# submarine0418/underwater_image_enhancement

Measured on AMD Instinct MI355X. Metric: megapixels/sec enhanced, higher is better.
Workload: dtype f32/f64

## Files before the change

include/uwie.h:

```cpp
#ifndef UWIE_H_
#define UWIE_H_

#include <stddef.h>
#include <stdint.h>

#ifdef __cplusplus
extern "C" {
#endif

#define UWIE_OK 0
#define UWIE_E_INVALID (-1)
#define UWIE_E_WORKSPACE (-2)
#define UWIE_E_HIP (-3)
#define UWIE_E_NODEVICE (-4)
#define UWIE_E_DEVICE (-5)

#define UWIE_SURFACE_SIX 0
#define UWIE_SURFACE_DICT 1

#define UWIE_DICT_STRONG_DEHAZING 0
#define UWIE_DICT_MEDIUM_DEHAZING 1
#define UWIE_DICT_LIGHT_ENHANCEMENT 2
#define UWIE_DICT_CLAHE_ENHANCEMENT 3
#define UWIE_DICT_HISTOGRAM_EQUALIZATION 4

#define UWIE_CAST_NORMAL 0
#define UWIE_CAST_GREENISH 1
#define UWIE_CAST_BLUISH 2

typedef struct uwie_ctx uwie_ctx;

typedef struct uwie_params {
    int32_t surface;
    int32_t strategy;
    int32_t cast_correct;
    int32_t forced_cast;
    int32_t gray_shift;
    int32_t min_size;
    double omega;
    int32_t gf_ksize;
    double gf_eps;
    double L_low, L_high;
    double wb_percentile;
    double clip_limit;
    int32_t tiles_x, tiles_y;
    double gamma;
    int32_t apply_gamma;
    int32_t gf_exact;
    int32_t inter_dtype;
    int32_t dark_patch;
} uwie_params;

#define UWIE_INTER_F64 0
#define UWIE_INTER_FX32 1
#define UWIE_INTER_F32T 2

const char *uwie_last_error(void);
const char *uwie_version(void);

int uwie_create(int device, uwie_ctx **out_ctx);
void uwie_destroy(uwie_ctx *ctx);

#define UWIE_STATUS_CANNY_LABEL 1u
#define UWIE_STATUS_FALLBACK_SYNC 2u
#define UWIE_STATUS_QTREE_BOUNDS 4u
#define UWIE_STATUS_FEATURE_COUNTS 8u
#define UWIE_STATUS_DIFF_RANK 16u
#define UWIE_STATUS_RESIZE_DESC 32u
#define UWIE_STATUS_CLASSIFY_NAN 64u
int uwie_device_status(uwie_ctx *ctx, void *stream, uint32_t *bits);

int uwie_profile_enable(uwie_ctx *ctx, int on);
int uwie_profile_filter(uwie_ctx *ctx, const char *kernel_name);
int uwie_profile_collect(uwie_ctx *ctx);
int uwie_profile_row(uwie_ctx *ctx, int i, const char **name, double *total_ms, int *calls);

int uwie_params_init(uwie_params *p, int surface, int strategy);

int uwie_set_tuning(uwie_ctx *ctx, const char *name, int value);
int uwie_get_tuning(uwie_ctx *ctx, const char *name, int *value);

size_t uwie_workspace_bytes(int batch, int H, int W, const uwie_params *p);
size_t uwie_workspace_bytes_ctx(uwie_ctx *ctx, int batch, int H, int W, const uwie_params *p);

int uwie_enhance_u8(uwie_ctx *ctx, const uint8_t *d_in, uint8_t *d_out_u8, float *d_out_f32, int batch, int H, int W,
                    const uwie_params *p, void *d_workspace, size_t workspace_bytes, void *stream);

int uwie_enhance_u8_f64(uwie_ctx *ctx, const uint8_t *d_in, uint8_t *d_out_u8, double *d_out_f64, int batch, int H, int W,
                        const uwie_params *p, void *d_workspace, size_t workspace_bytes, void *stream);

int uwie_enhance_percentiles(uwie_ctx *ctx, const void *d_workspace, size_t workspace_bytes, int batch, int H, int W,
                             const uwie_params *p, double *d_out, void *stream);

size_t uwie_workspace_bytes_float(int batch, int H, int W, const uwie_params *p, int elem_bytes);
int uwie_enhance_f32(uwie_ctx *ctx, const float *d_img, uint8_t *d_out_u8, float *d_out_f32, double *d_out_f64, int batch, int H, int W,
                     const uwie_params *p, void *d_workspace, size_t workspace_bytes, void *stream);
int uwie_enhance_f64(uwie_ctx *ctx, const double *d_img, uint8_t *d_out_u8, double *d_out_f64, int batch, int H, int W,
                     const uwie_params *p, void *d_workspace, size_t workspace_bytes, void *stream);
int uwie_cast_classify_f32(uwie_ctx *ctx, const float *d_img, int batch, int H, int W, int32_t *d_kind, float *d_mean_rgb, void *stream);
int uwie_color_correct_f32(uwie_ctx *ctx, const float *d_img, const int32_t *d_kind, float *d_out, int batch, int H, int W, void *stream);

size_t uwie_workspace_bytes_all(int batch, int H, int W, const uwie_params *p6);

int uwie_enhance_all_u8(uwie_ctx *ctx, const uint8_t *d_in, uint8_t *d_out_u8, int32_t *d_kind, int batch, int H, int W,
                        const uwie_params *p6, void *d_workspace, size_t workspace_bytes, void *stream);

#define UWIE_DIFF_OMEGA 1
#define UWIE_DIFF_GAMMA 2
int uwie_diff_enhance_f32(uwie_ctx *ctx, const float *d_img, float *d_out, int batch, int H, int W, int planar,
                          const float *d_params, int flags, void *d_workspace, size_t workspace_bytes, void *stream);

int uwie_diff_enhance_save_f32(uwie_ctx *ctx, const float *d_img, float *d_out, int batch, int H, int W, int planar,
                               const float *d_params, int flags, float *d_saved, void *d_workspace, size_t workspace_bytes,
                               void *stream);
size_t uwie_diff_enhance_bwd_workspace_bytes(int batch, int H, int W);
int uwie_diff_enhance_bwd_f32(uwie_ctx *ctx, const float *d_img, const float *d_params, int flags, int planar, int batch,
                              int H, int W, const float *d_saved, const float *d_grad_out, float *d_grad_img,
                              float *d_grad_params, void *d_workspace, size_t workspace_bytes, void *stream);

size_t uwie_workspace_bytes_diff_u8(int batch, int H, int W);
int uwie_diff_enhance_u8(uwie_ctx *ctx, const uint8_t *d_in, uint8_t *d_out_u8, float *d_out_f32, int batch, int H, int W,
                         const float *d_params ,
                         int flags , float *d_saved , void *d_workspace,
                         size_t workspace_bytes, void *stream);

int uwie_diff_gated_f32(uwie_ctx *ctx, const float *d_img, float *d_out, int batch, int H, int W, int planar,
                        const float *d_params, int flags, void *d_workspace, size_t workspace_bytes, void *stream);
int uwie_diff_gated_save_f32(uwie_ctx *ctx, const float *d_img, float *d_out, int batch, int H, int W, int planar,
                             const float *d_params, int flags, float *d_saved, void *d_workspace, size_t workspace_bytes,
                             void *stream);
size_t uwie_diff_gated_bwd_workspace_bytes(int batch, int H, int W);
int uwie_diff_gated_bwd_f32(uwie_ctx *ctx, const float *d_img, const float *d_params, int flags, int planar, int batch, int H,
                            int W, const float *d_saved, const float *d_grad_out, float *d_grad_img, float *d_grad_params,
                            void *d_workspace, size_t workspace_bytes, void *stream);

size_t uwie_workspace_bytes_diff_gated_u8(int batch);
int uwie_diff_gated_u8(uwie_ctx *ctx, const uint8_t *d_in, uint8_t *d_out_u8, float *d_out_f32, int batch, int H, int W,
                       const float *d_params , int flags ,
                       float *d_saved , void *d_workspace, size_t workspace_bytes, void *stream);

#define UWIE_LOSS_IDENTITY 0
#define UWIE_LOSS_VGG 1
#define UWIE_LOSS_GATED 2
size_t uwie_ref_loss_workspace_bytes(int batch, int H, int W);
int uwie_ref_loss_f32(uwie_ctx *ctx, int map, const float *d_img, const float *d_params, int flags, int planar, int batch, int H,
                      int W, const float *d_ref, float *d_out, float *d_saved, float *d_loss, void *d_workspace,
                      size_t workspace_bytes, void *stream);
int uwie_ref_loss_bwd_f32(uwie_ctx *ctx, int map, const float *d_img, const float *d_params, int flags, int planar, int batch,
                          int H, int W, const float *d_saved, const float *d_ref, const float *d_grad_out,
                          const float *d_grad_loss, float *d_grad_img, float *d_grad_params, void *d_workspace,
                          size_t workspace_bytes, void *stream);
int uwie_device_status_async(uwie_ctx *ctx, uint32_t *d_bits, void *stream);

// ... 207 lines not shown
```

underwater_image_enhancement_amd/_lib.py:

```python
from __future__ import annotations

import ctypes
import os
import subprocess

_HERE = os.path.dirname(os.path.abspath(__file__))
LIB_PATH = os.path.join(_HERE, "lib", "libuwie.so")
CSRC = os.path.join(_HERE, "csrc")

SURFACE_SIX, SURFACE_DICT = 0, 1
STATUS_DIFF_RANK = 16
STATUS_CLASSIFY_NAN = 64
LOSS_IDENTITY, LOSS_VGG, LOSS_GATED = 0, 1, 2
VGG_F32, VGG_F16, VGG_PARAMS = 0, 1, 1735488
PARAM_NET_PARAMS = {True: 8500100, False: 8459652}
MASKS_GIVEN, MASKS_DRAWN = 0, 1
TRAINER_PARAMS, TRAINER_GRADS, TRAINER_EXP_AVG, TRAINER_EXP_AVG_SQ = 0, 1, 2, 3
FLIP_LR, FLIP_UD = 1, 2
RESIZE_MAX_SIDE, RESIZE_MAX_SRC = 4096, 32768
INTER_F64, INTER_FX32, INTER_F32T = 0, 1, 2
DICT_STRATEGIES = {
    "strong_dehazing": 0,
    "medium_dehazing": 1,
    "light_enhancement": 2,
# ... 36 lines not shown
class UwieModelDesc(ctypes.Structure):

    _fields_ = [("kind", ctypes.c_int32), ("n_features", ctypes.c_int32), ("n_classes", ctypes.c_int32),
                ("n_trees", ctypes.c_int32), ("n_nodes", ctypes.c_int32), ("n_sv", ctypes.c_int32),
                ("mean", ctypes.c_void_p), ("scale", ctypes.c_void_p),
                ("tree_offset", ctypes.c_void_p), ("left", ctypes.c_void_p), ("right", ctypes.c_void_p),
                ("feature", ctypes.c_void_p), ("threshold", ctypes.c_void_p), ("missing_left", ctypes.c_void_p),
                ("value", ctypes.c_void_p), ("learning_rate", ctypes.c_double), ("init", ctypes.c_void_p),
                ("sv", ctypes.c_void_p), ("dual_coef", ctypes.c_void_p), ("intercept", ctypes.c_void_p),
                ("n_support", ctypes.c_void_p), ("prob_a", ctypes.c_void_p), ("prob_b", ctypes.c_void_p),
                ("gamma", ctypes.c_double)]


class UwieClahePlan(ctypes.Structure):

    _fields_ = [(name, ctypes.c_int32) for name in ("tile_w", "tile_h", "padded", "clip_limit", "wide_lut", "nchunk",
                                                    "cells_walk", "cells_flat")]


def clahe_plan(batch, H, W, tiles=(8, 8), clip_limit=2.0, recomputed=False) -> UwieClahePlan:
    out = UwieClahePlan()
    check(load().uwie_clahe_plan(batch, H, W, int(tiles[0]), int(tiles[1]), float(clip_limit), int(bool(recomputed)),
                                 ctypes.byref(out)))
    return out


def dark_patch_plan(H, W, k) -> tuple[int, int]:
    tw, th = ctypes.c_int(), ctypes.c_int()
    check(load().uwie_dark_patch_plan(int(H), int(W), int(k), ctypes.byref(tw), ctypes.byref(th)))
    return tw.value, th.value


UW_SCORES = 8


def underwater_plan(H, W) -> tuple[int, int]:
    tw, th = ctypes.c_int(), ctypes.c_int()
    check(load().uwie_underwater_plan(int(H), int(W), ctypes.byref(tw), ctypes.byref(th)))
    return tw.value, th.value


REF_SCORES = 8


def reference_plan(H, W) -> tuple[int, int]:
    tw, th = ctypes.c_int(), ctypes.c_int()
    check(load().uwie_reference_plan(int(H), int(W), ctypes.byref(tw), ctypes.byref(th)))
    return tw.value, th.value


GW_STATS = 12


def gray_world_plan(H, W) -> tuple[int, int]:
    bp, tp = ctypes.c_int(), ctypes.c_int()
    check(load().uwie_gray_world_plan(int(H), int(W), ctypes.byref(bp), ctypes.byref(tp)))
    return bp.value, tp.value


def fusion_plan(H, W, levels=1) -> tuple[int, int]:
    tw, th = ctypes.c_int(), ctypes.c_int()
    check(load().uwie_fusion_plan(int(H), int(W), int(levels), ctypes.byref(tw), ctypes.byref(th)))
    return tw.value, th.value


def fusion_table(gamma):
    import numpy as np

    buf = (ctypes.c_uint8 * 256)()
    check(load().uwie_fusion_table(float(gamma), buf))
    return np.frombuffer(bytes(buf), dtype=np.uint8).copy()


_VP, _SZ, _I, _D = ctypes.c_void_p, ctypes.c_size_t, ctypes.c_int, ctypes.c_double
_PP = ctypes.POINTER(UwieParams)
_PM = ctypes.POINTER(UwieModelDesc)
_PI = ctypes.POINTER(_I)
SIGNATURES = {
    "uwie_last_error": [],
    "uwie_version": [],
    "uwie_create": [_I, ctypes.POINTER(_VP)],
    "uwie_destroy": [_VP],
    "uwie_device_status": [_VP, _VP, ctypes.POINTER(ctypes.c_uint32)],
    "uwie_profile_enable": [_VP, _I],
    "uwie_profile_filter": [_VP, ctypes.c_char_p],
    "uwie_profile_collect": [_VP],
    "uwie_profile_row": [_VP, _I, ctypes.POINTER(ctypes.c_char_p), ctypes.POINTER(_D), ctypes.POINTER(_I)],
    "uwie_params_init": [_PP, _I, _I],
    "uwie_set_tuning": [_VP, ctypes.c_char_p, _I],
    "uwie_get_tuning": [_VP, ctypes.c_char_p, ctypes.POINTER(_I)],
    "uwie_workspace_bytes": [_I, _I, _I, _PP],
    "uwie_workspace_bytes_ctx": [_VP, _I, _I, _I, _PP],
    "uwie_workspace_bytes_all": [_I, _I, _I, _VP],
    "uwie_workspace_bytes_float": [_I, _I, _I, _PP, _I],
    "uwie_enhance_f32": [_VP, _VP, _VP, _VP, _VP, _I, _I, _I, _PP, _VP, _SZ, _VP],
    "uwie_enhance_f64": [_VP, _VP, _VP, _VP, _I, _I, _I, _PP, _VP, _SZ, _VP],
    "uwie_cast_classify_f32": [_VP, _VP, _I, _I, _I, _VP, _VP, _VP],
    "uwie_color_correct_f32": [_VP, _VP, _VP, _VP, _I, _I, _I, _VP],
    "uwie_guided_plan": [_I, _I, _I, _I, ctypes.POINTER(ctypes.c_int), ctypes.POINTER(ctypes.c_int)],
    "uwie_guided_fill": [_I, _I, _I, _I, ctypes.POINTER(ctypes.c_longlong)],
    "uwie_clahe_plan": [_I, _I, _I, _I, _I, _D, _I, ctypes.POINTER(UwieClahePlan)],
    "uwie_dark_patch_plan": [_I, _I, _I, ctypes.POINTER(ctypes.c_int), ctypes.POINTER(ctypes.c_int)],
    "uwie_enhance_u8": [_VP, _VP, _VP, _VP, _I, _I, _I, _PP, _VP, _SZ, _VP],
    "uwie_enhance_u8_f64": [_VP, _VP, _VP, _VP, _I, _I, _I, _PP, _VP, _SZ, _VP],
    "uwie_enhance_percentiles": [_VP, _VP, _SZ, _I, _I, _I, _PP, _VP, _VP],
    "uwie_enhance_all_u8": [_VP, _VP, _VP, _VP, _I, _I, _I, _VP, _VP, _SZ, _VP],
    "uwie_workspace_bytes_select": [_I, _I, _I, _VP, _I, _I],
    "uwie_select_best_u8": [_VP, _VP, _I, _I, _I, _VP, _I, _VP, _VP, _VP, _VP, _VP, _VP, _SZ, _VP],
    "uwie_workspace_bytes_underwater": [_I, _I, _I],
    "uwie_underwater_plan": [_I, _I, ctypes.POINTER(ctypes.c_int), ctypes.POINTER(ctypes.c_int)],
    "uwie_underwater_scores_u8": [_VP, _VP, _I, _I, _I, _I, _VP, _VP, _SZ, _VP],
    "uwie_workspace_bytes_reference": [_I, _I, _I],
    "uwie_reference_plan": [_I, _I, ctypes.POINTER(ctypes.c_int), ctypes.POINTER(ctypes.c_int)],
    "uwie_reference_scores_u8": [_VP, _VP, _VP, _I, _I, _I, _I, _I, _VP, _VP, _SZ, _VP],
    "uwie_workspace_bytes_gray_world": [_I, _I, _I],
    "uwie_gray_world_plan": [_I, _I, ctypes.POINTER(ctypes.c_int), ctypes.POINTER(ctypes.c_int)],
    "uwie_gray_world_u8": [_VP, _VP, _I, _I, _I, _D, _D, _D, _VP, _VP, _VP, _SZ, _VP],
    "uwie_workspace_bytes_fusion": [_I, _I, _I, _I],
    "uwie_fusion_plan": [_I, _I, _I, ctypes.POINTER(ctypes.c_int), ctypes.POINTER(ctypes.c_int)],
    "uwie_fusion_table": [_D, ctypes.POINTER(ctypes.c_uint8)],
    "uwie_fusion_u8": [_VP, _VP, _I, _I, _I, _D, _I, _I, _VP, _VP, _VP, _VP, _VP, _SZ, _VP],
    "uwie_pick_best_u8": [_VP, _VP, _I, _I, _I, _I, _VP, _I, _I, _VP, _VP, _VP],
    "uwie_diff_enhance_f32": [_VP, _VP, _VP, _I, _I, _I, _I, _VP, _I, _VP, _SZ, _VP],
    "uwie_diff_enhance_save_f32": [_VP, _VP, _VP, _I, _I, _I, _I, _VP, _I, _VP, _VP, _SZ, _VP],
    "uwie_diff_enhance_bwd_workspace_bytes": [_I, _I, _I],
    "uwie_workspace_bytes_diff_u8": [_I, _I, _I],
    "uwie_diff_enhance_u8": [_VP, _VP, _VP, _VP, _I, _I, _I, _VP, _I, _VP, _VP, _SZ, _VP],
    "uwie_diff_enhance_bwd_f32": [_VP, _VP, _VP, _I, _I, _I, _I, _I, _VP, _VP, _VP, _VP, _VP, _SZ, _VP],
    "uwie_diff_gated_f32": [_VP, _VP, _VP, _I, _I, _I, _I, _VP, _I, _VP, _SZ, _VP],
    "uwie_diff_gated_save_f32": [_VP, _VP, _VP, _I, _I, _I, _I, _VP, _I, _VP, _VP, _SZ, _VP],
    "uwie_diff_gated_bwd_workspace_bytes": [_I, _I, _I],
    "uwie_workspace_bytes_diff_gated_u8": [_I],
    "uwie_diff_gated_u8": [_VP, _VP, _VP, _VP, _I, _I, _I, _VP, _I, _VP, _VP, _SZ, _VP],
    "uwie_diff_gated_bwd_f32": [_VP, _VP, _VP, _I, _I, _I, _I, _I, _VP, _VP, _VP, _VP, _VP, _SZ, _VP],
    "uwie_ref_loss_workspace_bytes": [_I, _I, _I],
    "uwie_ref_loss_f32": [_VP, _I, _VP, _VP, _I, _I, _I, _I, _I, _VP, _VP, _VP, _VP, _VP, _SZ, _VP],
    "uwie_ref_loss_bwd_f32": [_VP, _I, _VP, _VP, _I, _I, _I, _I, _I, _VP, _VP, _VP, _VP, _VP, _VP, _VP, _SZ, _VP],
    "uwie_device_status_async": [_VP, _VP, _VP],
    "uwie_vgg_create": [_VP, _VP, _I, ctypes.POINTER(_VP)],
    "uwie_vgg_destroy": [_VP],
    "uwie_perceptual_workspace_bytes": [_I, _I, _I, _I],
    "uwie_perceptual_f32": [_VP, _VP, _VP, _VP, _I, _I, _I, _VP, _VP, _SZ, _VP],
    "uwie_perceptual_bwd_f32": [_VP, _VP, _I, _I, _I, _VP, _VP, _VP, _SZ, _VP],
    "uwie_param_net_create": [_VP, _VP, _I, ctypes.POINTER(_VP)],
    "uwie_param_net_destroy": [_VP],
    "uwie_param_net_workspace_bytes": [_I, _I, _I],
    "uwie_param_net_f32": [_VP, _VP, _VP, _VP, _I, _I, _I, _VP, _VP, _VP, _SZ, _VP],
    "uwie_mlp_create": [_VP, _VP, _I, _I, _I, ctypes.POINTER(_VP)],
    "uwie_mlp_destroy": [_VP],
    "uwie_mlp_workspace_bytes": [_I, _I],
    "uwie_mlp_forward": [_VP, _VP, _VP, _I, _I, _VP, _VP, _SZ, _VP],
    "uwie_mlp_trainer_create": [_VP, _VP, _I, _I, _I, ctypes.POINTER(_VP)],
    "uwie_mlp_trainer_destroy": [_VP],
    "uwie_mlp_train_workspace_bytes": [_I, _I, _I],
    "uwie_mlp_train_forward": [_VP, _VP, _VP, _I, _I, _D, _I, _VP, ctypes.c_uint64, _VP, _VP, _SZ, _VP],
    "uwie_mlp_backward": [_VP, _VP, _VP, _I, _I, _VP, _VP, _SZ, _VP],
    "uwie_mlp_adam_step": [_VP, _VP, _D, _D, _D, _D, _D, _VP, _VP],
    "uwie_mlp_trainer_get": [_VP, _I, _VP],
    "uwie_mlp_trainer_set": [_VP, _I, _VP],
    "uwie_mlp_trainer_step_count": [_VP],
    "uwie_mlp_trainer_set_step_count": [_VP, ctypes.c_longlong],
    "uwie_mlp_trainer_eval": [_VP, _VP, _VP, _I, _I, _VP, _VP, _SZ, _VP],
    "uwie_u8_to_f32": [_VP, _VP, _VP, _SZ, _VP],
    "uwie_extract_features_u8": [_VP, _VP, _VP, _I, _I, _I, _VP, _SZ, _VP],
    "uwie_feature_extractor_count": [_I, _I],
    "uwie_workspace_bytes_feature_extractor": [_I, _I, _I],
# ... 92 lines not shown
```

underwater_image_enhancement_amd/csrc/api.hip:

```cpp
#include <algorithm>
#include <cmath>
#include <cstdarg>
#include <cstdio>
#include <cstring>
#include <type_traits>

#include "common.h"

#include <cstdlib>

namespace uwie {

static thread_local char g_err[512] = "";
static thread_local uwie_ctx *g_ctx = nullptr;
static const Tuning g_default_tuning{};

const Tuning &tune() { return g_ctx ? g_ctx->tune : g_default_tuning; }
uwie_ctx *current_ctx() { return g_ctx; }

void set_error(const char *fmt, ...)
{
    va_list ap;
    va_start(ap, fmt);
    vsnprintf(g_err, sizeof g_err, fmt, ap);
// ... 191 lines not shown
    }
    size_scratch(u, s);
    return u;
}

Pipe carve_pipe(Carver &c, Shape s, const EnhancePlan &e)
{
    Pipe P{};
    const size_t n = (size_t)s.B * s.npx();
    P.kind = c.take<int32_t>(s.B);
    P.A = c.take<float>((size_t)s.B * 3);
    P.pct = c.take<float>((size_t)s.B * 3 * kMaxPct);
    P.guess = c.take<int32_t>(s.B);
    if (e.F64) {
        P.F64 = c.take<double>(n * 3);
        P.pct64 = c.take<double>((size_t)s.B * 3 * kMaxPct);
    }
    if (e.F) P.F = c.take<float>(n * 3);
    if (e.dehaze) {
        P.gray = c.take<uint8_t>(n);
        if (!e.t0_in_scratch) P.t0 = c.take<float>(n);
        P.t = c.take<double>(n);
    }
    P.scratch_bytes = e.scratch_bytes;
    P.scratch = c.take<char>(P.scratch_bytes);
    P.planes = e.guided.planes;
    if (e.t0_in_scratch) P.t0 = static_cast<float *>(P.scratch);
    if (e.qpart && P.scratch) P.qpart = reinterpret_cast<uint32_t *>(static_cast<char *>(P.scratch) + e.qoff);
    return P;
}

int stage_guided(const Pipe &P, Shape s, const EnhancePlan &e, const FuseT0Args &frame, hipStream_t st)
{
    const GuidedPlan &g = e.guided;
    UWIE_REQUIRE(!g.planes || (P.planes && P.t0 != P.scratch), "guided filter: the workspace layout has no planes for the exact-order filter");
    if (g.t0) UWIE_TRY(launch_t0(frame, e.dark_patch, s, P.t0, st));
    return launch_guided_plan(g, s, P.gray, P.t0, P.t, P.scratch, st, &frame);
}

int stretch_f32(const float *img, float *out, Shape s, double lo, double hi, float eps, float *pct, void *ws, hipStream_t st)
{
    const double q[2] = {lo, hi};
    UWIE_TRY(launch_percentiles(img, 0, s, q, 2, pct, ws, st));
    return launch_stretch_apply_f32(img, pct, 2, 0, 1, eps, out, s, st);
}

int six_cast(uwie_ctx *ctx, const uint8_t *d_in, Shape s, const EnhancePlan &e, const uwie_params *p, const Pipe &P,
             const int32_t **kind, hipStream_t st)
{
    *kind = nullptr;
    if (p->forced_cast >= 0) {
        UWIE_TRY(launch_set_kind(P.kind, s.B, p->forced_cast, st));
        *kind = P.kind;
    } else if (p->cast_correct) {
        const EntryFuse ef{P.qpart, e.cast_gray ? P.gray : nullptr, P.guess, p->gray_shift};
        UWIE_TRY(launch_cast_classify(ctx, d_in, s, P.kind, nullptr, P.scratch, st, e.qpart ? &ef : nullptr));
        *kind = P.kind;
    }
    return UWIE_OK;
}

int six_airlight(uwie_ctx *ctx, const uint8_t *d_in, const int32_t *kind, Shape s, const EnhancePlan &e, const uwie_params *p,
                 const Pipe &P, hipStream_t st)
{
    return launch_airlight(ctx, d_in, kind, P.gray, s, p->min_size, P.A, nullptr, P.scratch, st, e.cast_gray ? 0 : p->gray_shift,
                           e.qpart ? P.qpart : nullptr);
}

int six_dehaze_tail(uwie_ctx *ctx, const uint8_t *d_in, const int32_t *kind, Shape s, const EnhancePlan &e, const uwie_params *p,
                    const Pipe &P, uint8_t *d_out_u8, float *d_out_f32, hipStream_t st)
{
    const float eps = 1e-6f;
    const int k = p->strategy, nq = k == 3 ? 4 : 2, t_is_f32 = e.guided.t_f32;
    UWIE_TRY(stage_guided(P, s, e, FuseT0Args{d_in, kind, P.A, (float)p->omega, 1e-6f, 1}, st));
    SelectPlan plan;
    const double q[4] = {p->L_low, p->L_high, p->wb_percentile, 100 - p->wb_percentile};
    const RestoreSrc src{d_in, kind, P.A, P.t, t_is_f32};
    const RestoreSrc *recompute = e.store ? nullptr : &src;
    if (e.generic) {
        UWIE_TRY(select_begin<float>(s, q, nq, P.scratch, st, &plan));
        UWIE_TRY(launch_restore_planar_hist(d_in, kind, P.A, P.t, s, P.F, plan.ghist, st, false, nullptr, t_is_f32));
        UWIE_TRY(select_run(plan, P.F, 1, s, true, st));
    } else {
        UWIE_TRY(select_lin_begin<float>(s, q, nq, P.scratch, st, &plan, e.predict ? &src : nullptr));
        if (e.rank && plan.predicted) {
            UWIE_TRY(launch_restore_rank(src, s, plan, st));
            UWIE_TRY(select_rank_run(plan, s, st, src));
        } else {
            UWIE_TRY(launch_restore_planar_hist(d_in, kind, P.A, P.t, s, e.store ? P.F : nullptr, plan.ghist, st, true, &plan, t_is_f32));
            UWIE_TRY(select_lin_run(plan, P.F, s, st, recompute));
        }
    }
    if (k == 3) {
        UWIE_TRY(select_lerp_chain(plan, s, eps, P.pct, st));
        return launch_tail_plain(P.F, P.pct, 4, eps, 1, s, 0, 1.0, d_out_u8, d_out_f32, st);
    }
    UWIE_TRY(select_lerp(plan, s, P.pct, st));
    return launch_tail_clahe(ctx, P.F, P.pct, 2, eps, 0, s, p->clip_limit, e.tx, e.ty, k == 1 ? 1 : 0, p->gamma, d_out_u8, d_out_f32,
                             P.scratch, st, recompute);
}

int dict_dehaze(uwie_ctx *ctx, const uint8_t *d_in, Shape s, const EnhancePlan &e, const uwie_params *p, const Pipe &P,
                uint8_t *d_out_u8, float *d_out_f32, double *d_out_f64, hipStream_t st, bool have_airlight)
{
    if (!have_airlight)
        UWIE_TRY(launch_airlight(ctx, d_in, nullptr, P.gray, s, p->min_size, P.A, nullptr, P.scratch, st, p->gray_shift));
    UWIE_TRY(stage_guided(P, s, e, FuseT0Args{d_in, nullptr, P.A, (float)p->omega, 1e-10f, 0}, st));
    SelectPlan plan;
    const double q[2] = {p->L_low, p->L_high};
    const RestoreSrc src{d_in, nullptr, P.A, P.t};
    const RestoreSrc *recompute = e.store ? nullptr : &src;
    if (e.generic) {
        UWIE_TRY(select_begin<double>(s, q, 2, P.scratch, st, &plan));
        UWIE_TRY(launch_recover64_planar_hist(d_in, P.A, P.t, s, P.F64, plan.ghist, st));
        UWIE_TRY(select_run(plan, P.F64, 1, s, true, st));
    } else {
        UWIE_TRY(select_lin_begin<double>(s, q, 2, P.scratch, st, &plan, &src));
        UWIE_TRY(launch_recover64_planar_hist(d_in, P.A, P.t, s, e.store ? P.F64 : nullptr, plan.ghist, st, true, &plan));
        UWIE_TRY(select_lin_run(plan, P.F64, s, st, recompute));
    }
    UWIE_TRY(select_lerp(plan, s, P.pct64, st));
    return launch_tail_plain64(P.F64, P.pct64, s, p->apply_gamma, p->gamma, d_out_u8, d_out_f32, st, recompute, d_out_f64);
}

int run_enhance(uwie_ctx *ctx, const uint8_t *d_in, Shape s, const EnhancePlan &e, const uwie_params *p, const Pipe &P,
                uint8_t *d_out_u8, float *d_out_f32, double *d_out_f64, hipStream_t st, bool have_airlight = false)
{
    const int32_t *kind = nullptr;
    switch (e.pipeline) {
    case EP_SIX_DEHAZE:
        UWIE_TRY(six_cast(ctx, d_in, s, e, p, P, &kind, st));
        UWIE_TRY(six_airlight(ctx, d_in, kind, s, e, p, P, st));
        return six_dehaze_tail(ctx, d_in, kind, s, e, p, P, d_out_u8, d_out_f32, st);
    case EP_SIX_CODES:
        UWIE_TRY(six_cast(ctx, d_in, s, e, p, P, &kind, st));
        return launch_code_strategy(ctx, d_in, kind, s, p, d_out_u8, d_out_f32, P.scratch, st);
    case EP_DICT_DEHAZE: return dict_dehaze(ctx, d_in, s, e, p, P, d_out_u8, d_out_f32, d_out_f64, st, have_airlight);
    default: return launch_code_strategy(ctx, d_in, nullptr, s, p, d_out_u8, d_out_f32, P.scratch, st, d_out_f64);
    }
}

int check_params(const uwie_params *p)
{
    UWIE_REQUIRE(p != nullptr, "params is NULL");
    UWIE_REQUIRE(p->surface == UWIE_SURFACE_SIX || p->surface == UWIE_SURFACE_DICT, "unknown surface");
    if (p->surface == UWIE_SURFACE_SIX) UWIE_REQUIRE(p->strategy >= 1 && p->strategy <= 6, "unknown strategy");
    else UWIE_REQUIRE(p->strategy >= 0 && p->strategy <= 4, "unknown strategy");
    UWIE_REQUIRE(p->gray_shift == 14 || p->gray_shift == 15, "gray_shift must be 14 or 15");
    UWIE_REQUIRE(p->forced_cast >= -1 && p->forced_cast <= 2, "forced_cast must be -1 or a UWIE_CAST_* kind");
    UWIE_REQUIRE(p->min_size >= 1, "min_size must be >= 1");
    UWIE_REQUIRE(p->tiles_x >= 1 && p->tiles_y >= 1 && p->tiles_x * p->tiles_y <= 4096, "bad CLAHE tile grid");
    if (dehazes(p)) UWIE_REQUIRE(p->gf_ksize >= 1 && p->gf_ksize <= 1024, "guided-filter width out of range");
    UWIE_REQUIRE(p->L_low >= 0.0 && p->L_low <= 100.0 && p->L_high >= 0.0 && p->L_high <= 100.0,
                 "L_low / L_high must be percentiles in [0, 100]");
    if (p->surface == UWIE_SURFACE_SIX && (p->strategy >= 3 && p->strategy <= 5))
        UWIE_REQUIRE(p->wb_percentile >= 0.0 && p->wb_percentile <= 100.0, "wb_percentile must be in [0, 100]");
    UWIE_REQUIRE(p->inter_dtype == UWIE_INTER_F64 || p->inter_dtype == UWIE_INTER_FX32 || p->inter_dtype == UWIE_INTER_F32T,
                 "unknown inter_dtype");
    UWIE_REQUIRE(p->dark_patch >= 0 && p->dark_patch <= 31, "dark_patch must be 0 .. 31 (0 and 1: the per-pixel dark channel)");
    return UWIE_OK;
}


template <class T>
struct FloatPipe {
    int32_t *kind;
    T *A;
    float *pct;
// ... 211 lines not shown
const char *uwie_version(void) { return "uwie 0.1 (gfx950)"; }

int uwie_create(int device, uwie_ctx **out_ctx)
{
    UWIE_REQUIRE(out_ctx != nullptr, "out_ctx is NULL");
    *out_ctx = nullptr;
    int count = 0;
    if (hipGetDeviceCount(&count) != hipSuccess || count <= 0) {
        set_error("no HIP device available (libuwie has no CPU path)");
        return UWIE_E_NODEVICE;
    }
    UWIE_REQUIRE(device >= 0 && device < count, "device index out of range");
    UWIE_HIP_CHECK(hipSetDevice(device));
    int cus = 0;
    UWIE_HIP_CHECK(hipDeviceGetAttribute(&cus, hipDeviceAttributeMultiprocessorCount, device));
    uwie_ctx *ctx = new uwie_ctx();
    ctx->aux_ready = false;
    ctx->prof = prof_create();
    ctx->device = device;
    ctx->cus = cus;
    tuning_from_env(&ctx->tune);
    LabTables *lab = new LabTables();
    CastTables *cast = new CastTables();
    build_lab_tables(lab);
    build_cast_tables(cast);
    hipError_t e = hipMalloc((void **)&ctx->d_lab, sizeof(LabTables));
    if (e == hipSuccess) e = hipMalloc((void **)&ctx->d_cast, sizeof(CastTables));
    if (e == hipSuccess) e = hipMalloc((void **)&ctx->d_status, 64);
    if (e == hipSuccess) e = hipMemset(ctx->d_status, 0, 64);
    if (e == hipSuccess) e = hipMemcpy(ctx->d_lab, lab, sizeof(LabTables), hipMemcpyHostToDevice);
    if (e == hipSuccess) e = hipMemcpy(ctx->d_cast, cast, sizeof(CastTables), hipMemcpyHostToDevice);
    delete lab;
    delete cast;
    if (e != hipSuccess) {
        set_error("context table upload failed: %s", hipGetErrorString(e));
        uwie_destroy(ctx);
        return UWIE_E_HIP;
    }
    *out_ctx = ctx;
    return UWIE_OK;
}

void uwie_destroy(uwie_ctx *ctx)
{
    if (!ctx) return;
    if (ctx->d_lab) (void)hipFree(ctx->d_lab);
    if (ctx->d_cast) (void)hipFree(ctx->d_cast);
    if (ctx->d_status) (void)hipFree(ctx->d_status);
    if (ctx->aux_ready) {
        for (int i = 0; i < 4; ++i) {
            (void)hipStreamDestroy(ctx->aux[i]);
            (void)hipEventDestroy(ctx->join[i]);
        }
        (void)hipEventDestroy(ctx->fork);
    }
    prof_bind(nullptr);
    prof_destroy(ctx->prof);
    delete ctx;
}

int uwie_device_status(uwie_ctx *ctx, void *stream, uint32_t *bits)
{
    UWIE_REQUIRE(ctx != nullptr, "device_status: NULL context");
    UWIE_SCOPE(ctx);
    uint32_t v = 0;
    hipStream_t st = (hipStream_t)stream;
    UWIE_HIP_CHECK(hipMemcpyAsync(&v, ctx->d_status, sizeof v, hipMemcpyDeviceToHost, st));
    UWIE_HIP_CHECK(hipStreamSynchronize(st));
    if (v) UWIE_HIP_CHECK(hipMemsetAsync(ctx->d_status, 0, sizeof v, st));
    if (bits) *bits = v;
    if (v) {
        set_error("device status 0x%x:%s the results of the calls since the last check are not valid", v,
                  (v & UWIE_STATUS_CANNY_LABEL) ? " Canny hysteresis met a component label that this launch did not write (k_canny.hip);"
                  : (v & UWIE_STATUS_QTREE_BOUNDS) ? " a quadtree score fell outside its histogram interval (k_airlight.hip, tuning q_hist = 3);"
                  : (v & UWIE_STATUS_FEATURE_COUNTS) ? " a frame's feature histograms do not count every pixel (k_extractor.hip);"
                  : (v & UWIE_STATUS_DIFF_RANK) ? " a gated DifferentiableEnhancement image has no valid sorted position (an IndexError, ValueError or OverflowError in Python);"
                  : (v & UWIE_STATUS_RESIZE_DESC) ? " a resize frame descriptor has a NULL pointer or a size out of range (k_resize.hip);"
                  : (v & UWIE_STATUS_CLASSIFY_NAN) ? " a row holds NaN and the model is GB or SVC (scikit-learn: ValueError, Input X contains NaN);" : "");
        return UWIE_E_DEVICE;
    }
    return UWIE_OK;
}

int uwie_device_status_async(uwie_ctx *ctx, uint32_t *d_bits, void *stream)
{
    UWIE_REQUIRE(ctx && d_bits, "device_status_async: NULL pointer");
    UWIE_SCOPE(ctx);
    hipStream_t st = (hipStream_t)stream;
    UWIE_HIP_CHECK(hipMemcpyAsync(d_bits, ctx->d_status, sizeof(uint32_t), hipMemcpyDeviceToDevice, st));
    UWIE_HIP_CHECK(hipMemsetAsync(ctx->d_status, 0, sizeof(uint32_t), st));
    return UWIE_OK;
}

int uwie_profile_enable(uwie_ctx *ctx, int on)
{
    UWIE_REQUIRE(ctx != nullptr, "profile_enable: NULL context");
    prof_enable(ctx->prof, on != 0);
    prof_bind(on ? ctx->prof : nullptr);
    return UWIE_OK;
}

int uwie_profile_filter(uwie_ctx *ctx, const char *kernel_name)
{
    UWIE_REQUIRE(ctx != nullptr, "ctx is NULL");
    prof_filter(ctx->prof, kernel_name);
    return UWIE_OK;
}

int uwie_profile_collect(uwie_ctx *ctx)
{
    if (!ctx) {
        set_error("profile_collect: NULL context");
        return UWIE_E_INVALID;
    }
    return prof_collect(ctx->prof);
}

int uwie_profile_row(uwie_ctx *ctx, int i, const char **name, double *total_ms, int *calls)
{
    UWIE_REQUIRE(ctx && name && total_ms && calls, "profile_row: NULL pointer");
    return prof_row(ctx->prof, i, name, total_ms, calls);
}

int uwie_set_tuning(uwie_ctx *ctx, const char *name, int value)
{
    UWIE_REQUIRE(ctx && name, "set_tuning: NULL pointer");
    for (const KnobName &k : kKnobs)
        if (std::strcmp(k.name, name) == 0) {
            ctx->tune.*(k.field) = value;
            return UWIE_OK;
        }
    set_error("set_tuning: unknown selector '%s'", name);
    return UWIE_E_INVALID;
}

int uwie_get_tuning(uwie_ctx *ctx, const char *name, int *value)
{
    UWIE_REQUIRE(ctx && name && value, "get_tuning: NULL pointer");
    for (const KnobName &k : kKnobs)
        if (std::strcmp(k.name, name) == 0) {
            *value = ctx->tune.*(k.field);
            return UWIE_OK;
        }
    set_error("get_tuning: unknown selector '%s'", name);
    return UWIE_E_INVALID;
}

int uwie_params_init(uwie_params *p, int surface, int strategy)
{
    UWIE_REQUIRE(p != nullptr, "params is NULL");
    std::memset(p, 0, sizeof *p);
    p->surface = surface;
    p->strategy = strategy;
    p->gray_shift = 15;
    p->min_size = 1;
    p->tiles_x = p->tiles_y = 8;
    p->wb_percentile = -1.0;
    p->gamma = 1.2;
    p->forced_cast = -1;
    p->dark_patch = 1;
    if (surface == UWIE_SURFACE_SIX) {
        p->cast_correct = 1;
        switch (strategy) {
        case 1: p->omega = 0.3; p->gf_ksize = 20; p->gf_eps = 5e-1; p->L_low = 5; p->L_high = 98; p->clip_limit = 3.0; p->gamma = 1.5; p->apply_gamma = 1; break;
        case 2: p->omega = 0.5; p->gf_ksize = 15; p->gf_eps = 5e-1; p->L_low = 15; p->L_high = 95; p->clip_limit = 2.0; break;
        case 3: p->omega = 0.7; p->gf_ksize = 10; p->gf_eps = 1e-1; p->L_low = 20; p->L_high = 85; p->wb_percentile = 2; break;
// ... 1455 lines not shown
```

underwater_image_enhancement_amd/csrc/common.h:

```cpp
#pragma once
#include <hip/hip_runtime.h>
#include <stddef.h>
#include <stdint.h>

#include "../../include/uwie.h"

namespace uwie {

void set_error(const char *fmt, ...);
#define UWIE_HIP_CHECK(expr)                                                            \
    do {                                                                                \
        hipError_t _e = (expr);                                                         \
        if (_e != hipSuccess) {                                                         \
            ::uwie::set_error("%s failed: %s (%s:%d)", #expr, hipGetErrorString(_e), __FILE__, __LINE__); \
            return UWIE_E_HIP;                                                          \
        }                                                                               \
    } while (0)
#define UWIE_LAUNCH_CHECK() UWIE_HIP_CHECK(hipGetLastError())
#define UWIE_REQUIRE(cond, msg)                 \
    do {                                        \
        if (!(cond)) {                          \
            ::uwie::set_error("%s", msg);       \
            return UWIE_E_INVALID;              \
        }                                       \
    } while (0)

constexpr int kCastBinadeMin = -2;
constexpr int kCastBinades = 34;

struct LabTables {
    uint16_t gamma[256];
    uint16_t cbrt[3072];
    int32_t fwd[9];
    uint8_t invgamma[4096];
    int32_t ltoyf[512];
    int32_t abtoxz[36864];
    int32_t inv[9];
};

struct CastTables {
    uint32_t R[kCastBinades][256];
    uint8_t tie[kCastBinades][256];
    uint32_t RT[256][kCastBinades];
    uint2 RT2[128][kCastBinades];
    uint8_t tiebin[256];
};

void build_lab_tables(LabTables *t);
void build_cast_tables(CastTables *t);

struct Profiler;
Profiler *prof_create();
void prof_destroy(Profiler *p);
void prof_enable(Profiler *p, bool on);
void prof_filter(Profiler *p, const char *name);
void prof_bind(Profiler *p);
int prof_collect(Profiler *p);
int prof_row(Profiler *p, int i, const char **name, double *ms, int *calls);
class ProfScope {
public:
    ProfScope(const char *name, hipStream_t st);
    ~ProfScope();
    ProfScope(const ProfScope &) = delete;

private:
    int rec_;
    hipStream_t st_;
};
#define UWIE_PROF_CAT2(a, b) a##b
#define UWIE_PROF_CAT(a, b) UWIE_PROF_CAT2(a, b)
#define UWIE_PROF(name, st) ::uwie::ProfScope UWIE_PROF_CAT(_uwie_prof_, __LINE__)(name, st)
#define UWIE_LAUNCH_AS(row, kernel, grid, block, lds, st, ...)              \
    do {                                                                    \
        UWIE_PROF(row, st);                                                 \
        hipLaunchKernelGGL(kernel, grid, block, lds, st, __VA_ARGS__);      \
    } while (0)
#define UWIE_LAUNCH(kernel, ...) UWIE_LAUNCH_AS(#kernel, kernel, __VA_ARGS__)

}

namespace uwie {
struct Tuning {
    int gf_split = 1;
    int gf_bands = 0;
    int select_generic = 0;
    int restore_store = 0;
    int lin_predict3 = 0;
    int lin_cap = 0;
    int lin_no_predict = 0;
    int q_hist = 1;
    int lin_predict_shift = 0;
    int streams = 1;
    int canny_prepass = 1;
    int gf_fuse = 2;
    int rank_sweep = 1;
    int canny_fault_inject = 0;
    int entry_fuse = 1;
};
const Tuning &tune();
uwie_ctx *current_ctx();
}

struct uwie_ctx {
    int device;
    uwie::Tuning tune;
    bool attr_q_tail = false;
    bool attr_cast_resolve = false;
    int attr_gf_fast = 0;
    int attr_gf_split8 = 0;
    int cus = 0;
    uwie::LabTables *d_lab;
    uwie::CastTables *d_cast;
    uwie::Profiler *prof;
    uint32_t *d_status = nullptr;
    hipStream_t aux[4];
    hipEvent_t fork, join[4];
    bool aux_ready;
    bool last_enhance_f64 = false;
};

namespace uwie {

struct Carver {
    char *base;
    size_t off;
    explicit Carver(void *b) : base(static_cast<char *>(b)), off(0) {}
    template <typename T>
    T *take(size_t count)
    {
        off = (off + 255) & ~size_t(255);
        T *p = base ? reinterpret_cast<T *>(base + off) : nullptr;
        off += count * sizeof(T);
        return p;
    }
    size_t total() const { return (off + 255) & ~size_t(255); }
};

static inline int cdiv(long long a, long long b) { return (int)((a + b - 1) / b); }
static inline int grid_for(size_t n, size_t cap = 8192)
{
    size_t g = (n + 255) / 256;
    if (g > cap) g = cap;
    return g < 1 ? 1 : (int)g;
}

struct Region {
    int32_t img, y0, x0, rows, cols;
};

struct Shape {
    int B, H, W;
    size_t npx() const { return (size_t)H * W; }
};

size_t cast_ws_bytes(Shape s);
struct EntryFuse {
    uint32_t *qpart;
    uint8_t *gray;
    int32_t *guess;
    int gray_shift;
};
int launch_cast_classify(uwie_ctx *ctx, const uint8_t *d_in, Shape s, int32_t *d_kind, float *d_mean, void *ws,
                         hipStream_t st, const EntryFuse *ef = nullptr);
size_t quad_part_bytes(Shape s);
int launch_quad_hist_reduce(const uint32_t *qpart, Shape s, uint32_t *d_hist, hipStream_t st);
int launch_set_kind(int32_t *d_kind, int B, int kind, hipStream_t st);
int launch_normalise_correct(const uint8_t *d_in, const int32_t *d_kind, float *d_out, Shape s, hipStream_t st);
int launch_quant_gray(const uint8_t *d_in, const int32_t *d_kind, uint8_t *d_gray, Shape s, int gray_shift,
                      hipStream_t st);

size_t airlight_ws_bytes(Shape s);
int launch_airlight(uwie_ctx *ctx, const uint8_t *d_in, const int32_t *d_kind, uint8_t *d_gray, Shape s, int min_size,
                    float *d_A, void *d_trace, void *ws, hipStream_t st, int make_gray_shift = 0, const uint32_t *qpart = nullptr);
bool entry_fuse_takes(Shape s, int min_size);

size_t canny_ws_bytes(Shape s);
int launch_canny(const uint8_t *d_gray, Shape s, const Region *d_regions, int nreg, int max_rows, int max_cols, int low,
                 int high, uint32_t *d_count, uint8_t *d_edges, void *ws, hipStream_t st, bool count_is_zeroed = false,
                 bool strong_is_zeroed = false, bool prepass_done = false);
bool gray_strong_takes(Shape s);
int launch_gray_strong(const uint8_t *d_in, const int32_t *d_kind, uint8_t *d_gray, Shape s, const Region *d_regions, int nreg,
                       int max_rows, int max_cols, int high, int gray_shift, void *ws, hipStream_t st);
int launch_hist_strong(const uint8_t *d_in, const uint8_t *d_gray, Shape s, const Region *d_regions, int nreg, int max_rows,
                       int max_cols, int high, uint32_t *d_hist, void *ws, hipStream_t st);
uint32_t *canny_strong_flags(void *ws, Shape s);
int launch_make_full_regions(Region *d_regions, Shape s, hipStream_t st);

int launch_region_stats(const uint8_t *d_in, const int32_t *d_kind, const Region *d_regs, int nreg, int max_rows,
                        int max_cols, Shape s, float *csum, int maxChunks, float *tot, float *mean, float *vtot,
                        hipStream_t st);
int launch_frame_hist(const uint8_t *d_in, Shape s, uint32_t *d_hist, hipStream_t st);
size_t features_ws_bytes(Shape s);
// ... 57 lines not shown

size_t fusion_ws_bytes(Shape s, int levels);
void fusion_tile(int *tile_w, int *tile_h);
void fusion_table(double gamma, uint8_t *table256);
int launch_fusion(const uint8_t *d_in, Shape s, double gamma, int levels, int gray_shift, uint8_t *d_out, uint8_t *d_in1, uint8_t *d_in2,
                  double *d_weight, void *ws, hipStream_t st);

size_t guided_ws_bytes(Shape s);
size_t box_ws_bytes(Shape s);
int launch_trans_init(const uint8_t *d_in, const int32_t *d_kind, const float *d_A, Shape s, float omega, float norm_eps,
                      int pre_clip, float *d_t0, hipStream_t st);
int launch_box_filter_f64(const double *d_src, double *d_dst, Shape s, int k, void *ws, hipStream_t st);
int launch_trans_patch(const uint8_t *d_in, const int32_t *d_kind, const float *d_A, Shape s, int k, float omega, float norm_eps,
                       int pre_clip, float *d_t0, hipStream_t st);
void dark_patch_tile(int *tile_w, int *tile_h);
int launch_guided(const uint8_t *d_gray, const float *d_t0, Shape s, int k, double eps, double *d_t, void *ws,
                  hipStream_t st);
int launch_guided_p64(const uint8_t *d_gray, const double *d_t0, Shape s, int k, double eps, double *d_t, void *ws, hipStream_t st);

enum GuidedRoute {
    GF_EXACT,
    GF_FAST,
    GF_PIPE,
    GF_SPLIT,
    GF_FUSED,
};
struct GuidedRequest {
    int k;
    double eps;
    bool exact = false;
    bool fx = false;
    bool f32_ok = false;
    bool t0_from_frame = false;
    bool t0_f64 = false;
};
struct GuidedPlan {
    GuidedRoute route;
    int k;
    double eps;
    bool t_f32;
    bool ring_fx;
    bool t0_f64;
    bool t0;
    bool planes;
    int TH;
    int iy0, band, nb, rows;
    int pipe_bands;
};
GuidedPlan plan_guided(Shape s, const GuidedRequest &r);
inline long long guided_items(Shape s, const GuidedPlan &g) { return (long long)cdiv(s.W, 128 - 2 * (g.k - 1)) * g.nb * s.B; }
struct FuseT0Args {
    const uint8_t *rgb;
    const int32_t *kind;
    const float *A;
    float omega, norm_eps;
    int pre_clip;
};
int launch_guided_plan(const GuidedPlan &g, Shape s, const uint8_t *d_gray, const void *d_t0, double *d_t, void *ws, hipStream_t st,
                       const FuseT0Args *frame = nullptr);
int guided_fast_th(Shape s, int k);
int launch_guided_fast(const uint8_t *d_gray, const float *d_t0, Shape s, int k, int TH, double eps, double *d_t, hipStream_t st);

constexpr int kMaxPct = 4;
size_t select_ws_bytes(Shape s);
template <typename V>
int launch_percentiles(const V *d_vals, int planar, Shape s, const double *q_percent, int nq, V *d_out, void *ws, hipStream_t st);
int launch_widen_f32(const float *d_in, double *d_out, size_t n, hipStream_t st);

constexpr int kSelGroupStride = 2 * kMaxPct * 2048;
constexpr int kSelOsStride = 2 * kMaxPct;
struct LinState;
struct SelectPlan {
    void *state;
    uint32_t *ghist;
    void *os;
    double t[kMaxPct];
    int nq;
    bool is64;
    LinState *lin;
    void *lists;
    uint32_t *flags;
    uint32_t cap;
    bool predicted;
    uint32_t ranks[2 * kMaxPct];
    template <typename V>
    V *lists_as() const { return static_cast<V *>(lists); }
};
constexpr int kLinBins = 2050;
__host__ __device__ inline uint32_t lin_digit(float x)
{
    if (!(x > 0.0f)) return 0;
    if (x >= 1.0f) return kLinBins - 1;
    const uint32_t d = (uint32_t)(x * 2048.0f);
    return 1 + (d > 2047u ? 2047u : d);
}
__host__ __device__ inline uint32_t lin_digit(double x)
{
    if (!(x > 0.0)) return 0;
    if (x >= 1.0) return kLinBins - 1;
    const uint32_t d = (uint32_t)(x * 2048.0);
    return 1 + (d > 2047u ? 2047u : d);
}
constexpr int kLinLists = 2 * kMaxPct;
constexpr uint32_t kLinNoWin = 0x80000000u;
struct LinState {
    uint32_t rr[2 * kMaxPct];
    uint32_t qbin[2 * kMaxPct];
    uint32_t gid[2 * kMaxPct];
    uint32_t gbin[2 * kMaxPct];
    uint32_t gcount[kLinLists];
    uint32_t ngroups;
    uint32_t wlo[kMaxPct], wspan[kMaxPct];
    uint32_t below[kMaxPct];
};
constexpr int kRankCapMul = 4;
constexpr uint32_t kLinAnyBin = 0xfffffffeu;
struct RestoreSrc;
template <typename V>
int select_lin_begin(Shape s, const double *q_percent, int nq, void *ws, hipStream_t st, SelectPlan *plan,
                     const RestoreSrc *predict = nullptr);
template <typename V>
int select_lin_run(const SelectPlan &plan, const V *d_planar, Shape s, hipStream_t st, const RestoreSrc *src = nullptr);
template <typename V>
int select_begin(Shape s, const double *q_percent, int nq, void *ws, hipStream_t st, SelectPlan *plan);
template <typename V>
int select_run(const SelectPlan &plan, const V *d_vals, int planar, Shape s, bool pass1_done, hipStream_t st);
template <typename V>
int select_lerp(const SelectPlan &plan, Shape s, V *d_out, hipStream_t st);
int select_lerp_chain(const SelectPlan &plan, Shape s, float eps, float *d_pct4, hipStream_t st);
int select_begin_stretch_ranks(Shape s, const float *d_params, int stride, void *ws, hipStream_t st, SelectPlan *plan);
int select_begin_gated_ranks(Shape s, const float *d_params, int stride, uint32_t *d_status, void *ws, hipStream_t st,
                             SelectPlan *plan);
int launch_diff_enhance(const float *d_img, int planar, Shape s, const float *d_params, int flags, const float *d_os,
                        float *d_out, hipStream_t st, float *d_saved = nullptr);
size_t diff_u8_ws_bytes(Shape s);
int launch_diff_enhance_u8(const uint8_t *d_in, Shape s, const float *d_params, int flags, uint8_t *d_out_u8, float *d_out_f32,
                           float *d_saved, void *ws, hipStream_t st);
size_t diff_gated_u8_ws_bytes(int B);
int launch_diff_gated_u8(const uint8_t *d_in, Shape s, const float *d_params, uint32_t *d_status, uint8_t *d_out_u8,
                         float *d_out_f32, float *d_saved, void *ws, hipStream_t st);
int launch_diff_gated(const float *d_img, int planar, Shape s, const float *d_params, const float *d_os, float *d_out,
                      hipStream_t st, float *d_saved = nullptr);
size_t diff_enhance_bwd_ws_bytes(Shape s);
int launch_module_bwd(int map, const float *d_img, int planar, Shape s, const float *d_params, int flags, const float *d_saved,
                      const float *d_ref, const float *d_grad_out, const float *d_grad_loss, float *d_grad_img,
                      float *d_grad_params, void *ws, hipStream_t st);
size_t refloss_ws_bytes(Shape s);
int launch_refloss(int map, const float *d_img, int planar, Shape s, const float *d_params, int flags, const float *d_os,
                   const float *d_ref, float *d_out, float *d_saved, float *d_loss, void *ws, hipStream_t st);
int launch_refloss_bwd(int map, const float *d_img, int planar, Shape s, const float *d_params, int flags, const float *d_saved,
                       const float *d_ref, const float *d_grad_out, const float *d_grad_loss, float *d_grad_img,
                       float *d_grad_params, void *ws, hipStream_t st);
struct VggNet {
    int precision;
    const float *w0;
    const void *wf[7], *wb[7];
    const float *bias[7];
};
size_t vgg_param_count();
size_t vgg_blob_bytes(int precision);
int vgg_pack(const float *d_params, int precision, void *blob, VggNet *net, hipStream_t st);
size_t perceptual_ws_bytes(Shape s, int precision);
int launch_perceptual(const VggNet &net, const float *d_pred, const float *d_target, Shape s, float *d_loss, void *ws, hipStream_t st);
int launch_perceptual_bwd(const VggNet &net, Shape s, const float *d_grad_loss, float *d_grad_pred, void *ws, hipStream_t st);
int vgg_pack_conv_f32(const float *src, int Cout, int Cin, float *wf, float *wb_scratch, float *bias, hipStream_t st);
int launch_param_trunk(const VggNet &net, const float *const wf4[3], const float *const bias4[3], const float *img, Shape s, float *X,
                       float *Y, float **relu43, hipStream_t st);
struct ParamNet {
    VggNet trunk;
    const float *wf4[3], *bias4[3];
    int din;
    const float *lw[6], *lb[6];
    const float *bn[2];
};
size_t param_net_count(int use_features);
size_t param_net_blob_bytes(int use_features);
int param_net_pack(const float *d_params, int use_features, void *blob, float *scratch, ParamNet *net, hipStream_t st);
size_t param_net_scratch_floats();
size_t param_net_ws_bytes(Shape s);
int launch_param_net(const ParamNet &net, const float *img, const float *feat, Shape s, float *out, float *pooled, void *ws,
                     hipStream_t st);
int launch_u8_to_f32(const uint8_t *d_in, size_t n, float *d_out, hipStream_t st);
struct Mlp {
    int F, H, nb;
    const float *base;
    const float *hw, *hb;
};
size_t mlp_count(int F, int H, int nb);
int mlp_pack(const float *d_params, int F, int H, int nb, float *blob, Mlp *net, hipStream_t st);
size_t mlp_ws_bytes(int B, int hidden);
int launch_mlp(const Mlp &net, const void *feat, bool f64, int B, float *out, void *ws, hipStream_t st);
struct MlpAdam {
    float max_norm, w1, beta2, w2, bc2_sqrt, eps, neg_step;
};
size_t mlp_train_ws_bytes(int B, int hidden, int nb);
int mlp_train_sites(int nb);
int launch_mlp_train_forward(const Mlp &net, const void *feat, bool f64, int B, double p, const uint8_t *given, uint8_t *drawn_out,
                             uint64_t seed, uint32_t step, float *out, void *ws, hipStream_t st);
int launch_mlp_backward(const Mlp &net, float *grads, const void *feat, bool f64, int B, float scale, const float *grad_out, void *ws,
                        hipStream_t st);
size_t mlp_adam_scratch_bytes();
int launch_mlp_adam(const Mlp &net, float *params, float *grads, float *m, float *v, double *partial, const MlpAdam &h, double *norm_out,
                    hipStream_t st);
// ... 65 lines not shown
```

underwater_image_enhancement_amd/csrc/k_fused.hip:

```cpp
#include <cstdlib>

#include "common.h"
#include "devutil.h"
#include "restore.h"

namespace uwie {

namespace {


typedef float f32x2 __attribute__((ext_vector_type(2)));
#ifndef UWIE_CLAHE_PREFETCH
#define UWIE_CLAHE_PREFETCH 0
#endif
#ifndef UWIE_STRETCH_WAVES
#define UWIE_STRETCH_WAVES 5
#endif
#define UWIE_DESCALE(x, n) (((x) + (1 << ((n)-1))) >> (n))

template <bool LIN, bool COLLECT, int NW = 2, typename V = float>
__global__ void __launch_bounds__(256) k_restore_planar_hist(RestoreSrc S, int npx, V *__restrict__ planar,
                                                             uint32_t *__restrict__ ghist, LinState *__restrict__ lin,
                                                             V *__restrict__ lists, uint32_t cap)
{
// ... 156 lines not shown
                        old[c][i] = live && d - 1 < (uint32_t)kLinBins - 2 ? atomicAdd(&h[c][d], 1u) : 0u;
                    }
                if (COLLECT) {
#pragma unroll
                    for (int i = 0; i < 4; ++i)
#pragma unroll
                        for (int c = 0; c < 3; ++c)
                            if (old[c][i] >> kFlagShift) file(c, (int)(old[c][i] >> kFlagShift) - 1, r[c][i]);
                }
            } else if (ghist) {
#pragma unroll
                for (int i = 0; i < 4; ++i) {
                    if (i < n) {
#pragma unroll
                        for (int c = 0; c < 3; ++c) {
                            if constexpr (F64) bump(c, (uint32_t)(f64_key(r[c][i]) >> 53));
                            else bump(c, f32_key(r[c][i]) >> 21);
                        }
                    }
                }
            }
            if (planar) {
                if constexpr (F64) {
                    if (aligned && n == 4) {
                        V *o[3] = {o0, o1, o2};
#pragma unroll
                        for (int c = 0; c < 3; ++c) {
                            *reinterpret_cast<double2 *>(o[c] + p) = make_double2(r[c][0], r[c][1]);
                            *reinterpret_cast<double2 *>(o[c] + p + 2) = make_double2(r[c][2], r[c][3]);
                        }
                    } else {
                        for (int i = 0; i < n; ++i) {
                            o0[p + i] = r[0][i];
                            o1[p + i] = r[1][i];
                            o2[p + i] = r[2][i];
                        }
                    }
                } else if (aligned && n == 4) {
                    *reinterpret_cast<float4 *>(o0 + p) = make_float4(r[0][0], r[0][1], r[0][2], r[0][3]);
                    *reinterpret_cast<float4 *>(o1 + p) = make_float4(r[1][0], r[1][1], r[1][2], r[1][3]);
                    *reinterpret_cast<float4 *>(o2 + p) = make_float4(r[2][0], r[2][1], r[2][2], r[2][3]);
                } else {
                    for (int i = 0; i < n; ++i) {
                        o0[p + i] = r[0][i];
                        o1[p + i] = r[1][i];
                        o2[p + i] = r[2][i];
                    }
                }
            }
        }
        if (COLLECT && (it & 7) == 7) flush(false);
    }
    if (!ghist) return;
    if (COLLECT) flush(true);
#pragma unroll
    for (int c = 0; c < 3; ++c) {
        if (run[c]) atomicAdd(&h[c][cur[c]], run[c]);
        if (LIN) {
            const uint32_t z = wave_sum_u32(sat0[c]), o = wave_sum_u32(sat1[c]);
            if ((tid & 63) == 0) {
                if (z) atomicAdd(&h[c][0], z);
                if (o) atomicAdd(&h[c][kLinBins - 1], o);
            }
        }
    }
    __syncthreads();
    for (int i = tid; i < 3 * NB; i += 256) {
        const uint32_t c = (&h[0][0])[i] & (COLLECT ? kCntMask : 0xffffffffu);
        if (c) atomicAdd(&ghist[(size_t)(b * 3 + i / NB) * kSelGroupStride + (i % NB)], c);
    }
    };
    if constexpr (FAST) {
        if (S.t32) {
            RestoreImgT<2, true> R;
            sweep(R);
            return;
        }
    }
    RestoreImgT<FAST ? 2 : 0> R;
    sweep(R);
}

constexpr float kRankMargin = 1e-5f;
constexpr int kRankNW = 2, kRankNS = 3 * kRankNW;
constexpr int kRankQW = 64 + 64 * 12;
constexpr int kRankSW = 128;

struct RankWave {
    const uint8_t *img;
    const double *t;
    const float *ftab;
    float a0, a1, a2;
    const uint32_t *s_wlo, *s_wspan;
    const float *s_lo, *s_hi;
    uint32_t *s_below;
    uint32_t *myq;
    float (*mystg)[kRankSW];
    uint32_t *gcount0;
    uint32_t gstride;
    float *lists0;
    uint32_t cap;
    int lane;
};

__device__ __forceinline__ void rank_flush_stage(const RankWave &X, int j, uint32_t &scj)
{
    const uint32_t n = scj;
    const int c = j / kRankNW, w = j % kRankNW;
    uint32_t base = 0;
    if (X.lane == 0) base = atomicAdd(X.gcount0 + (size_t)c * X.gstride + w, n);
    base = (uint32_t)__builtin_amdgcn_readfirstlane((int)base);
    float *L = X.lists0 + ((size_t)c * (kLinLists / kRankCapMul) + w) * X.cap;
    wave_lds_sync();
    for (uint32_t i = X.lane; i < n; i += 64)
        if (base + i < X.cap) L[base + i] = X.mystg[j][i];
    wave_lds_sync();
    scj = 0;
}

__device__ __forceinline__ void rank_exact_batch(const RankWave &X, uint32_t first, uint32_t m, bool counted, uint32_t (&sc)[kRankNS])
{
    wave_lds_sync();
    int jj = -1;
    float x = 0.0f;
    if ((uint32_t)X.lane < m) {
        const uint32_t e = X.myq[first + X.lane];
        const int p = (int)(e >> 2), c = (int)(e & 3u);
        const double tv = X.t[p];
        const uint32_t u = X.img[(size_t)p * 3 + c];
        const float df = X.ftab[c * 256 + (int)u], ac = c == 0 ? X.a0 : c == 1 ? X.a1 : X.a2;
        const double n = (double)df;
        double q;
        if (RestoreImgT<1>::recip_ok(tv)) {
            const double y = RestoreImgT<1>::recip(tv), q0 = n * y;
            q = fma(fma(-tv, q0, n), y, q0);
        } else {
            q = n / tv;
        }
        x = clip01((float)(q + (double)ac));
        const uint32_t d = lin_digit(x);
        const float v32 = fmaf(df, __builtin_amdgcn_rcpf((float)tv), ac);
#pragma unroll
        for (int w = 0; w < kRankNW; ++w) {
            const int j = c * kRankNW + w;
            const uint32_t wlo = X.s_wlo[j];
            if (wlo == kLinNoWin) continue;
            if (counted && !(v32 >= X.s_lo[j] && v32 <= X.s_hi[j])) continue;
            if (d < wlo) atomicAdd(&X.s_below[j], 1u);
            else if (d - wlo <= X.s_wspan[j]) jj = j;
        }
    }
#pragma unroll
    for (int j = 0; j < kRankNS; ++j) {
        const uint64_t mk = __ballot(jj == j);
        if (mk) {
            const uint32_t pos = sc[j] + (uint32_t)__popcll(mk & ((1ull << X.lane) - 1));
            if (jj == j) X.mystg[j][pos] = x;
            sc[j] += (uint32_t)__popcll(mk);
            if (sc[j] >= 64u) rank_flush_stage(X, j, sc[j]);
        }
    }
}

__global__ void __launch_bounds__(256) k_restore_rank(RestoreSrc S, int npx, LinState *__restrict__ lin, float *__restrict__ lists,
                                                      uint32_t cap)
{
    constexpr int NW = kRankNW, NS = kRankNS, QW = kRankQW, SW = kRankSW;
    __shared__ uint32_t wq[4][QW];
    __shared__ float wstg[4][NS][SW];
    __shared__ float ftab[768];
    __shared__ uint32_t s_wlo[NS], s_wspan[NS];
    __shared__ float s_lo[NS], s_hi[NS];
    __shared__ uint32_t s_below[NS];
    const int b = blockIdx.y, tid = threadIdx.x, lane = tid & 63, wv = tid >> 6;
    if (tid < NS) {
        s_below[tid] = 0;
        const LinState &L = lin[3 * b + tid / NW];
        const uint32_t lo = L.wlo[tid % NW], span = L.wspan[tid % NW];
        s_wlo[tid] = lo;
        s_wspan[tid] = span;
        s_lo[tid] = lo == kLinNoWin ? __builtin_inff() : (float)(lo - 1) * (1.0f / 2048.0f) - kRankMargin;
        s_hi[tid] = lo == kLinNoWin ? -__builtin_inff() : (float)(lo + span) * (1.0f / 2048.0f) + kRankMargin;
    }
    RestoreImgT<1> R;
    R.init(S, b, (size_t)npx, ftab);
    __syncthreads();
    float elo[NS], ehi[NS];
#pragma unroll
    for (int j = 0; j < NS; ++j) {
        elo[j] = s_lo[j];
        ehi[j] = s_hi[j];
    }
    const float a0 = R.a[0], a1 = R.a[1], a2 = R.a[2];
    const uint8_t *img = S.in + (size_t)b * npx * 3;
    const double *tpl = S.t + (size_t)b * npx;
    uint32_t *myq = wq[wv];
    uint32_t cnt[NS] = {0, 0, 0, 0, 0, 0};
    uint32_t seen = 0;
    uint32_t qn = 0;
    uint32_t sc[NS] = {0, 0, 0, 0, 0, 0};

    const RankWave X{img, tpl, ftab, a0, a1, a2, s_wlo, s_wspan, s_lo, s_hi, s_below, myq, wstg[wv],
                     &lin[3 * b].gcount[0], (uint32_t)(sizeof(LinState) / sizeof(uint32_t)),
                     lists + (size_t)(3 * b) * (kLinLists / kRankCapMul) * cap, cap, lane};

    const int step = gridDim.x * 1024, iters = (npx + step - 1) / step;
#define UWIE_RANK_LOAD4(p_, w_, tv_)                                                                                   \
    do {                                                                                                                \
        const u32_unaligned *q_ = reinterpret_cast<const u32_unaligned *>(img + (size_t)(p_) * 3);                      \
        (w_)[0] = q_[0]; (w_)[1] = q_[1]; (w_)[2] = q_[2];                                                              \
        const double2_a8 ta_ = *reinterpret_cast<const double2_a8 *>(tpl + (p_)),                                       \
                         tb_ = *reinterpret_cast<const double2_a8 *>(tpl + (p_) + 2);                                   \
        (tv_)[0] = ta_.x; (tv_)[1] = ta_.y; (tv_)[2] = tb_.x; (tv_)[3] = tb_.y;                                         \
    } while (0)
    uint32_t w_nx[3] = {0, 0, 0};
    double tv_nx[4] = {1.0, 1.0, 1.0, 1.0};
    bool have_nx = false;
    const int p_last = npx - 4;
    {
        const int p0 = (blockIdx.x * 256 + tid) * 4;
        have_nx = p0 + 4 <= npx;
        UWIE_RANK_LOAD4(min(p0, p_last), w_nx, tv_nx);
    }
    for (int it = 0; it < iters; ++it) {
        const int p = it * step + (blockIdx.x * 256 + tid) * 4;
        const bool have = have_nx;
        const uint32_t w0 = w_nx[0], w1 = w_nx[1], w2 = w_nx[2];
        const double tv[4] = {tv_nx[0], tv_nx[1], tv_nx[2], tv_nx[3]};
        {
            const int pn = p + step;
            have_nx = it + 1 < iters && pn + 4 <= npx;
            UWIE_RANK_LOAD4(min(pn, p_last), w_nx, tv_nx);
        }
        uint32_t fm = 0;
        seen += 4u * (uint32_t)__popcll(__ballot(have));
        if (have) {
            float y[4];
#pragma unroll
            for (int i = 0; i < 4; ++i) y[i] = __builtin_amdgcn_rcpf((float)tv[i]);
            const uint32_t ub[3][4] = {{w0 & 255, w0 >> 24, (w1 >> 16) & 255, (w2 >> 8) & 255},
                                       {(w0 >> 8) & 255, w1 & 255, w1 >> 24, (w2 >> 16) & 255},
                                       {(w0 >> 16) & 255, (w1 >> 8) & 255, w2 & 255, w2 >> 24}};
#pragma unroll
            for (int c = 0; c < 3; ++c) {
                const float ac = c == 0 ? a0 : c == 1 ? a1 : a2;
#pragma unroll
                for (int i = 0; i < 4; ++i) {
                    const float v = fmaf(ftab[c * 256 + (int)ub[c][i]], y[i], ac);
                    bool in = false;
#pragma unroll
                    for (int w = 0; w < NW; ++w) {
                        const bool ge = v >= elo[c * NW + w];
                        cnt[c * NW + w] += (uint32_t)__popcll(__ballot(ge));
                        in = in | (ge & (v <= ehi[c * NW + w]));
                    }
                    fm |= (uint32_t)in << (4 * c + i);
                }
                __builtin_amdgcn_sched_barrier(0);
            }
        }
        const bool ragged = !have && p < npx;
        const uint32_t nmine = (uint32_t)__popc(fm);
        if (__ballot(nmine != 0)) {
            uint32_t pre = 0, tot = 0;
#pragma unroll
            for (int bit = 0; bit < 4; ++bit) {
                const uint64_t mk = __ballot((nmine >> bit) & 1u);
                pre += (uint32_t)__popcll(mk & ((1ull << lane) - 1)) << bit;
                tot += (uint32_t)__popcll(mk) << bit;
            }
            uint32_t at = qn + pre;
            for (uint32_t f = fm; f; f &= f - 1, ++at) {
                const int k = __ffs(f) - 1;
                myq[at] = ((uint32_t)(p + (k & 3)) << 2) | (uint32_t)(k >> 2);
            }
            qn += tot;
            while (qn >= 64u) {
                qn -= 64u;
                rank_exact_batch(X, qn, 64u, true, sc);
            }
        }
        if (__ballot(ragged)) {
            const uint32_t n3 = ragged ? (uint32_t)(npx - p) * 3u : 0u;
            wave_lds_sync();
            if (ragged)
                for (uint32_t i = 0; i < n3; ++i) myq[qn + i] = ((uint32_t)(p + (int)(i / 3u)) << 2) | (i % 3u);
            const uint32_t m = (uint32_t)__builtin_amdgcn_readfirstlane((int)__shfl((int)n3, (int)__builtin_ctzll(__ballot(ragged))));
// ... 755 lines not shown
    }
    L.wide = recomputed && (long)tx * ty * s.B < 512 && (long)g.tw * g.th >= 8192;
    L.cells = (tx + 1) * (ty + 1);
#ifndef UWIE_APPLY_TOTAL
#define UWIE_APPLY_TOTAL 25920
#endif
    const int nchunk = cdiv(UWIE_APPLY_TOTAL, L.cells * s.B);
    L.nchunk = std::max(1, std::min(nchunk, std::max(1, g.th / 16)));
    return L;
}

float gamma_exponent(int mode, double g) { return mode == 1 ? (float)g : mode == 2 ? (float)(1.0 / g) : 1.0f; }

int producer_blocks(int total, Shape s)
{
    const int nblk = std::min(std::max(cdiv(total, s.B), 16), 384);
    return std::min(nblk, cdiv((long long)s.npx(), 1024));
}

template <typename V>
struct HistRows;
template <>
struct HistRows<float> {
    static constexpr const char *collect = "k_restore_hist_collect", *collect4 = "k_restore_hist_collect4", *lin = "k_restore_hist_lin",
                                *key = "k_restore_hist_key", *plan_msg = "restore: a selection plan goes with its own linear histogram";
};
template <>
struct HistRows<double> {
    static constexpr const char *collect = "k_recover64_hist_collect", *collect4 = collect, *lin = "k_recover64_hist_lin",
                                *key = "k_recover64_hist_key", *plan_msg = "recover: a selection plan goes with its own linear histogram";
};

template <typename V>
int launch_planar_hist(const RestoreSrc &S, Shape s, V *d_planar, uint32_t *d_ghist, hipStream_t st, bool linear, const SelectPlan *plan)
{
    using Rows = HistRows<V>;
    constexpr bool f64 = sizeof(V) == 8;
    constexpr int NW4 = f64 ? 2 : 4;
    if (plan) UWIE_REQUIRE(linear && d_ghist == plan->ghist && (!f64 || plan->nq <= 2), Rows::plan_msg);
    const dim3 grid(producer_blocks(12288, s), s.B);
    const auto launch = [&](const char *row, auto kernel) {
        UWIE_LAUNCH_AS(row, kernel, grid, dim3(256), 0, st, S, (int)s.npx(), d_planar, d_ghist, plan ? plan->lin : nullptr,
                       plan ? plan->lists_as<V>() : nullptr, plan ? plan->cap : 0u);
    };
    if (plan && plan->nq <= 2) launch(Rows::collect, k_restore_planar_hist<true, true, 2, V>);
    else if (plan) launch(Rows::collect4, k_restore_planar_hist<true, true, NW4, V>);
    else if (linear) launch(Rows::lin, k_restore_planar_hist<true, false, 2, V>);
    else launch(Rows::key, k_restore_planar_hist<false, false, 2, V>);
    UWIE_LAUNCH_CHECK();
    return UWIE_OK;
}

}

void clahe_plan_info(Shape s, double clip, int tx, int ty, bool recomputed, uwie_clahe_plan_info *out)
{
    const ClaheLaunch L = plan_clahe(s, clip, tx, ty, recomputed);
    const ClaheGeom &g = L.g;
    out->tile_w = g.tw;
    out->tile_h = g.th;
    out->padded = L.padded;
    out->clip_limit = g.clip;
    out->wide_lut = L.wide;
    out->nchunk = L.nchunk;
    out->cells_walk = out->cells_flat = 0;
    int rows = 0;
    for (int cyi = 0; cyi <= ty; ++cyi)
        rows += std::max(cyi * g.th - g.th / 2, 0) < std::min((cyi + 1) * g.th - g.th / 2, g.H);
    for (int cxi = 0; cxi <= tx; ++cxi) {
        const int cx0 = std::max(cxi * g.tw - g.tw / 2, 0), cx1 = std::min((cxi + 1) * g.tw - g.tw / 2, g.W);
        if (cx0 >= cx1) continue;
        (clahe_apply_walks((cx1 - cx0 + 3) / 4) ? out->cells_walk : out->cells_flat) += rows;
    }
}

int launch_restore_planar_hist(const uint8_t *d_in, const int32_t *d_kind, const float *d_A, const double *d_t, Shape s,
                               float *d_planar, uint32_t *d_ghist, hipStream_t st, bool linear, const SelectPlan *plan, int t32)
{
    return launch_planar_hist<float>(RestoreSrc{d_in, d_kind, d_A, d_t, t32}, s, d_planar, d_ghist, st, linear, plan);
}

int launch_restore_rank(const RestoreSrc &src, Shape s, const SelectPlan &plan, hipStream_t st)
{
    UWIE_REQUIRE(!src.t32 && plan.nq <= 2 && plan.predicted && s.npx() >= 4, "restore_rank: float64 transmission, two predicted percentiles");
    UWIE_LAUNCH(k_restore_rank, dim3(producer_blocks(5120, s), s.B), dim3(256), 0, st, src, (int)s.npx(), plan.lin, plan.lists_as<float>(),
                (uint32_t)kRankCapMul * plan.cap);
    UWIE_LAUNCH_CHECK();
    return UWIE_OK;
}

int launch_recover64_planar_hist(const uint8_t *d_in, const float *d_A, const double *d_t, Shape s, double *d_planar,
                                 uint32_t *d_ghist, hipStream_t st, bool linear, const SelectPlan *plan)
{
    return launch_planar_hist<double>(RestoreSrc{d_in, nullptr, d_A, d_t}, s, d_planar, d_ghist, st, linear, plan);
}

int launch_tail_plain64(const double *d_planar, const double *d_pct, Shape s, int apply_gamma, double gamma,
                        uint8_t *d_out_u8, float *d_out_f32, hipStream_t st, const RestoreSrc *src, double *d_out_f64)
{
    const dim3 grid(grid_for(s.npx(), 4096), s.B);
    if (src)
        UWIE_LAUNCH(k_stretch64_out<true>, grid, dim3(256), 0, st, d_planar, *src, d_pct, (int)s.npx(), apply_gamma, 1.0 / gamma,
                    d_out_u8, d_out_f32, d_out_f64);
    else
        UWIE_LAUNCH(k_stretch64_out<false>, grid, dim3(256), 0, st, d_planar, RestoreSrc{}, d_pct, (int)s.npx(), apply_gamma,
                    1.0 / gamma, d_out_u8, d_out_f32, d_out_f64);
    UWIE_LAUNCH_CHECK();
    return UWIE_OK;
}

size_t tail_ws_bytes(Shape s, int tx, int ty)
{
    Carver c(nullptr);
    c.take<uint8_t>((size_t)s.B * tx * ty * 256);
    c.take<uint8_t>((size_t)s.B * s.npx() * 3);
    return c.total();
}

int launch_tail_clahe(uwie_ctx *ctx, const float *d_planar, const float *d_pct, int pct_stride, float eps, int two,
                      Shape s, double clip, int tx, int ty, int gamma_mode, double gamma, uint8_t *d_out_u8,
                      float *d_out_f32, void *ws, hipStream_t st, const RestoreSrc *src)
{
    Carver c(ws);
    uint8_t *lut = c.take<uint8_t>((size_t)s.B * tx * ty * 256);
    uint8_t *lab = c.take<uint8_t>((size_t)s.B * s.npx() * 3);
    const ClaheLaunch L = plan_clahe(s, clip, tx, ty, src != nullptr);
    const ClaheGeom &g = L.g;
    const auto k_stretch_lab_lut_wide = k_stretch_lab_lut<1, 1024>;
    if (L.wide)
        UWIE_LAUNCH(k_stretch_lab_lut_wide, dim3(tx * ty, s.B), dim3(1024), 0, st, ctx->d_lab, d_planar, *src, d_pct, pct_stride,
                    eps, two, (const uint8_t *)nullptr, g, lab, lut);
    else if (src)
        UWIE_LAUNCH(k_stretch_lab_lut<1>, dim3(tx * ty, s.B), dim3(256), 0, st, ctx->d_lab, d_planar, *src, d_pct, pct_stride,
                    eps, two, (const uint8_t *)nullptr, g, lab, lut);
    else
        UWIE_LAUNCH(k_stretch_lab_lut<0>, dim3(tx * ty, s.B), dim3(256), 0, st, ctx->d_lab, d_planar, RestoreSrc{}, d_pct,
                    pct_stride, eps, two, (const uint8_t *)nullptr, g, lab, lut);
    UWIE_LAUNCH_CHECK();
    const int cells = L.cells, nchunk = L.nchunk;
    const auto k_clahe_apply_u8 = k_clahe_apply_out<false, false>;
    const auto k_clahe_apply_f32 = k_clahe_apply_out<false, true>;
    if (d_out_f32)
        UWIE_LAUNCH(k_clahe_apply_f32, dim3(cells * nchunk, s.B), dim3(256), 0, st, ctx->d_lab, lab, lut, g, nchunk, gamma_mode,
                    gamma_exponent(gamma_mode, gamma), (const uint8_t *)nullptr, (const float *)nullptr, d_out_u8, d_out_f32,
                    (uint8_t *)nullptr, (uint32_t *)nullptr);
    else
        UWIE_LAUNCH(k_clahe_apply_u8, dim3(cells * nchunk, s.B), dim3(256), 0, st, ctx->d_lab, lab, lut, g, nchunk, gamma_mode,
                    gamma_exponent(gamma_mode, gamma), (const uint8_t *)nullptr, (const float *)nullptr, d_out_u8, d_out_f32,
                    (uint8_t *)nullptr, (uint32_t *)nullptr);
    UWIE_LAUNCH_CHECK();
    return UWIE_OK;
}

int launch_clahe_apply_codes(uwie_ctx *ctx, const uint8_t *d_lab, const uint8_t *d_tile_lut, Shape s, double clip, int tx,
                             int ty, const uint8_t *d_fin_code, const float *d_fin_val, uint8_t *d_out_u8, float *d_out_f32,
                             uint8_t *d_codes_out, uint32_t *d_hist, hipStream_t st)
{
    const ClaheLaunch L = plan_clahe(s, clip, tx, ty, false);
    const ClaheGeom &g = L.g;
    const int cells = L.cells, nchunk = L.nchunk;
    const auto k_clahe_apply_codes = k_clahe_apply_out<true, false>;
    UWIE_LAUNCH(k_clahe_apply_codes, dim3(cells * nchunk, s.B), dim3(256), 0, st, ctx->d_lab, d_lab, d_tile_lut, g, nchunk, 0, 1.0f,
                d_fin_code, d_fin_val, d_out_u8, d_out_f32, d_codes_out, d_hist);
    UWIE_LAUNCH_CHECK();
    return UWIE_OK;
}

int launch_codes_lab_lut(uwie_ctx *ctx, const uint8_t *d_in, const uint8_t *d_code_lut, Shape s, double clip, int tx, int ty,
                         uint8_t *d_lab, uint8_t *d_tile_lut, hipStream_t st)
// ... 21 lines not shown
```

underwater_image_enhancement_amd/csrc/k_select.hip:

```cpp
#include <cmath>
#include <cstdlib>

#include "common.h"
#include "devutil.h"
#include "restore.h"

namespace uwie {

namespace {

constexpr int kMaxRanks = 2 * kMaxPct;
constexpr int kBins = 2048;

template <typename V>
struct Traits;
template <>
struct Traits<float> {
    using K = uint32_t;
    static constexpr int NPASS = 3;
    __host__ __device__ static int shift(int p) { return p == 0 ? 21 : p == 1 ? 10 : 0; }
    __host__ __device__ static int bits(int p) { return p == 2 ? 10 : 11; }
    __device__ static K key(float v) { return f32_key(v); }
    __device__ static float value(K k) { return __uint_as_float(k ^ ((k >> 31) ? 0x80000000u : 0xffffffffu)); }
};
// ... 300 lines not shown
        const size_t lds = (size_t)(p == 0 ? 1 : nq) * (1u << Traits<V>::bits(p)) * sizeof(uint32_t);
        UWIE_LAUNCH(k_sel_pass<Src>, dim3(sweep ? blocks : 1, nbc), dim3(256), lds, st, src, n, (SelState<K> *)plan.state, p, nq,
                    sweep, plan.ghist, (V *)plan.os, only);
        UWIE_LAUNCH_CHECK();
    }
    return UWIE_OK;
}

int pass_blocks(long long n, int nbc, bool recomputed)
{
    if (recomputed) return 96;
    int blocks = (int)((n + 262143) / 262144);
    if (blocks * nbc < 256) blocks = cdiv(256, nbc);
    return std::max(1, std::min(blocks, 256));
}
template <typename V>
__device__ __forceinline__ V np_lerp(V a, V b, V t)
{
    const V diff = b - a;
    V r = a + diff * t;
    if (t >= (V)0.5) r = b - diff * ((V)1 - t);
    return r;
}

template <typename V>
__global__ void k_pct_finish(const V *__restrict__ os, int nbc, FracList<V> fr, V *__restrict__ out)
{
    const int i = blockIdx.x * blockDim.x + threadIdx.x;
    if (i >= nbc * fr.n) return;
    const int bc = i / fr.n, j = i % fr.n;
    out[i] = np_lerp<V>(os[bc * kMaxRanks + 2 * j], os[bc * kMaxRanks + 2 * j + 1], fr.t[j]);
}

__global__ void k_pct_finish_chain(const float *__restrict__ os, int nbc, FracList<float> fr, float eps,
                                   float *__restrict__ out)
{
    const int bc = blockIdx.x * blockDim.x + threadIdx.x;
    if (bc >= nbc) return;
    const float *o = os + bc * kMaxRanks;
    const float lo1 = np_lerp<float>(o[0], o[1], fr.t[0]), hi1 = np_lerp<float>(o[2], o[3], fr.t[1]);
    const float den = (hi1 - lo1) + eps;
    float m[4];
    for (int i = 0; i < 4; ++i) m[i] = fminf(fmaxf((o[4 + i] - lo1) / den, 0.0f), 1.0f);
    out[bc * 4 + 0] = lo1;
    out[bc * 4 + 1] = hi1;
    out[bc * 4 + 2] = np_lerp<float>(m[0], m[1], fr.t[2]);
    out[bc * 4 + 3] = np_lerp<float>(m[2], m[3], fr.t[3]);
}

template <typename V>
void percentile_indices(long long n, double q_percent, uint32_t *prev, uint32_t *next, double *t)
{
    const V q = (V)q_percent / (V)100;
    const V nm1 = (V)(n - 1);
    const V vi = nm1 * q;
    const V p = std::floor(vi);
    if (vi >= nm1) {
        *prev = *next = (uint32_t)(n - 1);
        *t = 0.0;
        return;
    }
    *prev = (uint32_t)p;
    *next = *prev + 1;
    *t = (double)(vi - p);
}

uint32_t lin_cap(Shape s)
{
    const uint32_t dflt = (uint32_t)std::max<size_t>(65536, s.npx() / 64);
    const long v = tune().lin_cap;
    return v > 0 && v < (long)dflt ? (uint32_t)v : dflt;
}

void carve_select(Carver &c, Shape s, bool lin, SelectPlan *plan)
{
    const size_t nbc = (size_t)s.B * 3;
    plan->state = c.take<SelState<uint64_t>>(nbc);
    plan->ghist = c.take<uint32_t>(nbc * kMaxRanks * kBins);
    plan->os = c.take<double>(nbc * kMaxRanks);
    if (!lin) return;
    plan->lin = c.take<LinState>(nbc);
    plan->flags = c.take<uint32_t>(nbc);
    plan->cap = lin_cap(s);
    plan->lists = c.take<double>(nbc * kLinLists * plan->cap);
}

int zero_ghist(const SelectPlan &plan, Shape s, hipStream_t st)
{
    UWIE_HIP_CHECK(hipMemsetAsync(plan.ghist, 0, sizeof(uint32_t) * (size_t)s.B * 3 * kMaxRanks * kBins, st));
    return UWIE_OK;
}

RankList rank_list(const SelectPlan &plan)
{
    RankList ranks;
    ranks.n = 2 * plan.nq;
    for (int j = 0; j < ranks.n; ++j) ranks.r[j] = plan.ranks[j];
    return ranks;
}

template <typename V>
int plan_percentiles(Shape s, const double *q_percent, int nq, void *ws, bool lin, SelectPlan *plan)
{
    UWIE_REQUIRE(nq >= 1 && nq <= kMaxPct, "percentiles: 1..4 percentiles per call");
    const long long n = (long long)s.npx();
    UWIE_REQUIRE(n >= 1 && n < (1ll << 31), "percentiles: plane size out of range");
    Carver c(ws);
    carve_select(c, s, lin, plan);
    plan->nq = nq;
    plan->is64 = sizeof(V) == 8;
    for (int j = 0; j < nq; ++j)
        percentile_indices<V>(n, q_percent[j], &plan->ranks[2 * j], &plan->ranks[2 * j + 1], &plan->t[j]);
    return UWIE_OK;
}

__global__ void k_sel_init_stretch_ranks(SelState<uint32_t> *st, int nbc, const float *__restrict__ params, int stride,
                                         int n)
{
    const int i = blockIdx.x * blockDim.x + threadIdx.x;
    if (i >= nbc) return;
    const float *pr = params + (size_t)(i / 3) * stride;
    RankList ranks;
    ranks.n = 2;
    for (int q = 0; q < 2; ++q) {
        const double pos = ((double)pr[q] / 100.0) * (double)n;
        long long idx = (long long)pos;
        idx = idx < 0 ? 0 : idx > n - 1 ? n - 1 : idx;
        ranks.r[q] = (uint32_t)idx;
    }
    st[i] = sel_state<uint32_t>(ranks);
}

__global__ void k_sel_init_gated_ranks(SelState<uint32_t> *st, int nbc, const float *__restrict__ params, int stride, int n,
                                       uint32_t *status)
{
    const int i = blockIdx.x * blockDim.x + threadIdx.x;
    if (i >= nbc) return;
    const float *pr = params + (size_t)(i / 3) * stride;
    int k[2];
    const bool ok0 = gated_rank(pr[0], n, &k[0]), ok1 = gated_rank(pr[1], n, &k[1]);
    const bool ok = ok0 && ok1;
    RankList ranks;
    ranks.n = 2;
    ranks.r[0] = ok ? (uint32_t)k[0] : 0u;
    ranks.r[1] = ok ? (uint32_t)k[1] : 0u;
    if (!ok && status) atomicOr(status, (uint32_t)UWIE_STATUS_DIFF_RANK);
    st[i] = sel_state<uint32_t>(ranks);
}

template <class Init>
int begin_ranks(Shape s, const char *range_msg, void *ws, hipStream_t st, SelectPlan *plan, Init &&init)
{
    const long long n = (long long)s.npx();
    UWIE_REQUIRE(n >= 1 && n < (1ll << 31), range_msg);
    Carver c(ws);
    carve_select(c, s, false, plan);
    plan->nq = 1;
    plan->is64 = false;
    plan->t[0] = 0.0;
    init((SelState<uint32_t> *)plan->state, s.B * 3, (int)n);
    UWIE_LAUNCH_CHECK();
    return zero_ghist(*plan, s, st);
}

}

namespace {

constexpr uint32_t kLinDone = 0xffffffffu;
constexpr int kLinSampleOff = 4096;

template <typename V>
__global__ void __launch_bounds__(256) k_lin_sample(RestoreSrc S, int npx, int stride, int ngs, uint32_t *__restrict__ ghist)
{
    __shared__ uint32_t h[3][kLinBins];
    const int b = blockIdx.y, tid = threadIdx.x;
    for (int i = tid; i < 3 * kLinBins; i += 256) (&h[0][0])[i] = 0;
    __syncthreads();
    RestoreImg R;
    RestoreImg32 R32;
    if (S.t32) R32.init(S, b, (size_t)npx);
    else R.init(S, b, (size_t)npx);
    for (int i = blockIdx.x * 256 + tid; i < ngs; i += gridDim.x * 256) {
        V r[3][4];
        if constexpr (sizeof(V) == 8) R.four64((i * stride + stride / 2) * 4, 4, r);
        else if (S.t32) R32.four((i * stride + stride / 2) * 4, 4, r);
        else R.four((i * stride + stride / 2) * 4, 4, r);
#pragma unroll
        for (int c = 0; c < 3; ++c)
#pragma unroll
            for (int j = 0; j < 4; ++j) atomicAdd(&h[c][lin_digit(r[c][j])], 1u);
    }
    __syncthreads();
    for (int i = tid; i < 3 * kLinBins; i += 256) {
        const uint32_t c = (&h[0][0])[i];
        if (c) atomicAdd(&ghist[(size_t)(b * 3 + i / kLinBins) * kSelGroupStride + kLinSampleOff + (i % kLinBins)], c);
    }
}

__global__ void __launch_bounds__(256) k_lin_predict(LinState *__restrict__ st, uint32_t *__restrict__ ghist,
                                                     RankList ranks, uint32_t n, uint32_t ns, int shift)
{
    __shared__ uint32_t h[kLinBins], wsum[4], found[2], wl[kMaxPct], wh[kMaxPct];
    const int bc = blockIdx.x, tid = threadIdx.x;
    if (tid < kMaxPct) { wl[tid] = kLinNoWin; wh[tid] = 0; }
    if (ns > 0) {
        uint32_t *gh = ghist + (size_t)bc * kSelGroupStride + kLinSampleOff;
        for (int i = tid; i < kLinBins; i += 256) {
            h[i] = gh[i];
            gh[i] = 0;
        }
        __syncthreads();
        for (int j = 0; j < ranks.n / 2 && j < kMaxPct; ++j) {
            const double p = (double)ranks.r[2 * j] / (double)n, sd = sqrt((double)ns * p * (1.0 - p));
            const double c0 = (double)ranks.r[2 * j] * ns / n, c1 = (double)ranks.r[2 * j + 1] * ns / n, delta = 4.0 * sd + 2.0;
            const uint32_t rlo = (uint32_t)fmax(c0 - delta, 0.0), rhi = (uint32_t)fmin(c1 + delta, (double)ns - 1.0);
            uint32_t dlo, dhi, rr;
            block_find_digit(h, kLinBins, rlo, wsum, found, dlo, rr);
            block_find_digit(h, kLinBins, rhi, wsum, found, dhi, rr);
            if (tid == 0) {
                wl[j] = (uint32_t)min(max((int)dlo + shift, 1), kLinBins - 2);
                wh[j] = (uint32_t)min(max((int)dhi + shift, (int)wl[j]), kLinBins - 2);
            }
        }
    }
    __syncthreads();
    if (tid == 0) {
        LinState s;
        for (int q = 0; q < kMaxRanks; ++q) { s.rr[q] = 0; s.qbin[q] = 0; s.gid[q] = kLinDone; s.gbin[q] = kLinDone; }
        for (int g = 0; g < kLinLists; ++g) s.gcount[g] = 0;
        s.ngroups = 0;
        for (bool again = true; again;) {
            again = false;
            for (int i = 0; i < kMaxPct; ++i)
                for (int j = i + 1; j < kMaxPct; ++j)
                    if (wl[i] != kLinNoWin && wl[j] != kLinNoWin && wl[j] <= wh[i] + 1 && wl[i] <= wh[j] + 1) {
                        wl[i] = min(wl[i], wl[j]);
                        wh[i] = max(wh[i], wh[j]);
                        wl[j] = kLinNoWin;
                        again = true;
                    }
        }
        for (int w = 0; w < kMaxPct; ++w) {
            s.wlo[w] = wl[w];
            s.wspan[w] = wl[w] == kLinNoWin ? 0 : wh[w] - wl[w];
            s.below[w] = 0;
        }
        st[bc] = s;
    }
}

template <typename V>
__global__ void __launch_bounds__(256) k_lin_scan(LinState *__restrict__ st, uint32_t *__restrict__ ghist, RankList ranks,
                                                  V *__restrict__ os, uint32_t *__restrict__ flags, uint32_t cap,
                                                  SelState<typename Traits<V>::K> *__restrict__ sel)
{
    __shared__ uint32_t h[kLinBins], wsum[4], found[2], qbin[kMaxRanks], qrr[kMaxRanks];
    const int bc = blockIdx.x, tid = threadIdx.x;
    if (tid == 0) sel[bc] = sel_state<typename Traits<V>::K>(ranks);
    uint32_t *gh = ghist + (size_t)bc * kSelGroupStride;
    for (int i = tid; i < kLinBins; i += 256) {
        h[i] = gh[i];
        gh[i] = 0;
    }
    __syncthreads();
    for (int q = 0; q < ranks.n; ++q) {
        uint32_t d, rr;
        block_find_digit(h, kLinBins, ranks.r[q], wsum, found, d, rr);
        if (tid == 0) { qbin[q] = d; qrr[q] = rr; }
    }
    __syncthreads();
    if (tid == 0) {
        LinState s = st[bc];
        bool covered = true;
        for (int q = 0; q < kMaxRanks; ++q) { s.rr[q] = 0; s.qbin[q] = 0; s.gid[q] = kLinDone; s.gbin[q] = kLinDone; }
        for (int q = 0; q < ranks.n; ++q) {
            s.rr[q] = qrr[q];
            s.qbin[q] = qbin[q];
            if (qbin[q] == 0 || qbin[q] == kLinBins - 1) {
                os[bc * kMaxRanks + q] = qbin[q] == 0 ? (V)0 : (V)1;
                continue;
            }
            int w = -1;
            for (int i = kMaxPct - 1; i >= 0; --i)
                if (qbin[q] - s.wlo[i] <= s.wspan[i]) w = i;
            if (w >= 0 && s.gcount[w] > cap) w = -1;
            if (w >= 0) s.gid[q] = (uint32_t)w;
            else covered = false;
        }
        uint32_t ng = 0;
        if (!covered) {
            for (int g = 0; g < kLinLists; ++g) s.gcount[g] = 0;
            for (int q = 0; q < ranks.n; ++q) {
                s.gid[q] = kLinDone;
                if (qbin[q] == 0 || qbin[q] == kLinBins - 1) continue;
                uint32_t g = 0;
                for (; g < ng; ++g)
                    if (s.gbin[g] == qbin[q]) break;
                if (g == ng) s.gbin[ng++] = qbin[q];
                s.gid[q] = g;
            }
        }
        s.ngroups = ng;
        st[bc] = s;
        flags[bc] = 0;
    }
}

__global__ void k_rank_scan(LinState *__restrict__ st, RankList ranks, float *__restrict__ os, uint32_t *__restrict__ flags,
                            uint32_t cap, int nbc, SelState<uint32_t> *__restrict__ sel)
{
    const int bc = blockIdx.x * blockDim.x + threadIdx.x;
    if (bc >= nbc) return;
    sel[bc] = sel_state<uint32_t>(ranks);
    LinState s = st[bc];
    bool miss = false;
    for (int q = 0; q < kMaxRanks; ++q) { s.rr[q] = 0; s.qbin[q] = 0; s.gid[q] = kLinDone; s.gbin[q] = kLinDone; }
    for (int q = 0; q < ranks.n; ++q) {
        const uint32_t r = ranks.r[q];
        bool done = false;
        for (int w = 0; w < kMaxPct && !done; ++w) {
            if (s.wlo[w] == kLinNoWin) continue;
            const uint32_t below = s.below[w], cnt = s.gcount[w];
            if (r >= below && r - below < cnt) {
                if (cnt <= cap) {
                    s.gid[q] = (uint32_t)w;
                    s.rr[q] = r - below;
                    s.qbin[q] = kLinAnyBin;
                } else {
                    miss = true;
                }
                done = true;
            } else if (r < below && s.wlo[w] == 1u) {
                os[bc * kMaxRanks + q] = 0.0f;
                done = true;
            } else if (r >= below && s.wlo[w] + s.wspan[w] == (uint32_t)kLinBins - 2u) {
                os[bc * kMaxRanks + q] = 1.0f;
                done = true;
            }
        }
        miss = miss || !done;
    }
    s.ngroups = 0;
    st[bc] = s;
    flags[bc] = miss ? 1u : 0u;
}

template <typename V>
__global__ void __launch_bounds__(256) k_lin_collect(const V *__restrict__ vals, int n, LinState *__restrict__ st,
                                                     V *__restrict__ lists, uint32_t cap)
{
    constexpr int kStage = sizeof(V) == 8 ? 256 : 512;
    __shared__ V stg[kMaxRanks][kStage];
    __shared__ uint32_t scount[kMaxRanks], sbase[kMaxRanks];
    const int bc = blockIdx.y, tid = threadIdx.x;
    LinState *s = st + bc;
    const int ng = (int)s->ngroups;
    if (ng == 0) return;
    uint32_t gd[kMaxRanks];
#pragma unroll
    for (int g = 0; g < kMaxRanks; ++g) gd[g] = g < ng ? s->gbin[g] - 1 : kLinDone;
    if (tid < kMaxRanks) scount[tid] = 0;
    __syncthreads();
    V *L = lists + (size_t)bc * kLinLists * cap;
    const V *v = vals + (size_t)bc * n;
    const int per = (((n + 3) / 4 + gridDim.x - 1) / gridDim.x) * 4;
    const int lo = min(n, blockIdx.x * per), hi = min(n, lo + per);
    auto take = [&](V x, bool live) {
        const uint32_t d = (live && x > (V)0) ? (uint32_t)(x * (V)2048) : 0xfffffffeu;
        uint32_t idx = kLinDone;
#pragma unroll
        for (int g = 0; g < 4; ++g) idx = d == gd[g] ? (uint32_t)g : idx;
        if (ng > 4) {
#pragma unroll
            for (int g = 4; g < kMaxRanks; ++g) idx = d == gd[g] ? (uint32_t)g : idx;
        }
        if (idx != kLinDone) {
            const uint32_t pos = atomicAdd(&scount[idx], 1u);
            if (pos < (uint32_t)kStage) {
                stg[idx][pos] = x;
            } else {
                const uint32_t at = atomicAdd(&s->gcount[idx], 1u);
                if (at < cap) L[(size_t)idx * cap + at] = x;
            }
        }
    };
    auto flush = [&](bool force) {
        __syncthreads();
        bool need = force;
        for (int g = 0; g < ng; ++g) need = need || scount[g] > (uint32_t)(kStage * 3 / 4);
        if (!need) return;
        if (tid < ng) sbase[tid] = atomicAdd(&s->gcount[tid], min(scount[tid], (uint32_t)kStage));
        __syncthreads();
        for (int g = 0; g < ng; ++g) {
            const uint32_t c = min(scount[g], (uint32_t)kStage), base = sbase[g];
            for (uint32_t i = tid; i < c; i += 256)
                if (base + i < cap) L[(size_t)g * cap + base + i] = stg[g][i];
        }
        __syncthreads();
        if (tid < kMaxRanks) scount[tid] = 0;
        __syncthreads();
    };
    const bool vec = ((size_t)v & 15) == 0;
    const int hiv = vec ? lo + ((hi - lo) / 4) * 4 : lo;
    constexpr int U = sizeof(V) == 8 ? 2 : 4;
    for (int base = lo; base < hiv; base += U * 1024) {
        const int i = base + tid * 4;
        V raw[U][4];
        bool ok[U];
#pragma unroll
        for (int u = 0; u < U; ++u) {
            ok[u] = i + u * 1024 < hiv;
            if constexpr (sizeof(V) == 8) {
                const double2 lo2 = ok[u] ? *reinterpret_cast<const double2 *>(v + i + u * 1024) : make_double2(0, 0);
                const double2 hi2 = ok[u] ? *reinterpret_cast<const double2 *>(v + i + u * 1024 + 2) : make_double2(0, 0);
                raw[u][0] = lo2.x; raw[u][1] = lo2.y; raw[u][2] = hi2.x; raw[u][3] = hi2.y;
            } else {
                const float4 q = ok[u] ? *reinterpret_cast<const float4 *>(v + i + u * 1024) : make_float4(0, 0, 0, 0);
                raw[u][0] = q.x; raw[u][1] = q.y; raw[u][2] = q.z; raw[u][3] = q.w;
            }
        }
#pragma unroll
        for (int u = 0; u < U; ++u) {
#pragma unroll
            for (int e = 0; e < 4; ++e) take(raw[u][e], ok[u]);
        }
        flush(false);
    }
// ... 11 lines not shown
{
    constexpr int kStage = sizeof(V) == 8 ? 256 : 512;
    __shared__ V stg[3 * NG][kStage];
    __shared__ uint32_t scount[3 * NG], sbase[3 * NG];
    const int b = blockIdx.y, tid = threadIdx.x;
    LinState *s = st + 3 * b;
    int ngc[3];
    uint32_t gd[3][NG];
#pragma unroll
    for (int c = 0; c < 3; ++c) {
        ngc[c] = min((int)s[c].ngroups, NG);
#pragma unroll
        for (int g = 0; g < NG; ++g) gd[c][g] = g < ngc[c] ? s[c].gbin[g] - 1 : kLinDone;
    }
    if (ngc[0] + ngc[1] + ngc[2] == 0) return;
    if (tid < 3 * NG) scount[tid] = 0;
    __syncthreads();
    RestoreImg R;
    RestoreImg32 R32;
    if (S.t32) R32.init(S, b, (size_t)n);
    else R.init(S, b, (size_t)n);
    const int per = (((n + 3) / 4 + gridDim.x - 1) / gridDim.x) * 4;
    const int lo = min(n, blockIdx.x * per), hi = min(n, lo + per);
    auto take = [&](int c, V x, bool live) {
        const uint32_t d = (live && x > (V)0) ? (uint32_t)(x * (V)2048) : 0xfffffffeu;
        uint32_t idx = kLinDone;
#pragma unroll
        for (int g = 0; g < NG; ++g) idx = d == gd[c][g] ? (uint32_t)g : idx;
        if (idx != kLinDone) {
            const uint32_t pos = atomicAdd(&scount[c * NG + idx], 1u);
            if (pos < (uint32_t)kStage) {
                stg[c * NG + idx][pos] = x;
            } else {
                const uint32_t at = atomicAdd(&s[c].gcount[idx], 1u);
                if (at < cap) lists[((size_t)(3 * b + c) * kLinLists + idx) * cap + at] = x;
            }
        }
    };
    auto flush = [&](bool force) {
        __syncthreads();
        bool need = force;
        for (int j = 0; j < 3 * NG; ++j) need = need || scount[j] > (uint32_t)(kStage * 3 / 4);
        if (!need) return;
        if (tid < 3 * NG) {
            const uint32_t c = min(scount[tid], (uint32_t)kStage);
            if (c) sbase[tid] = atomicAdd(&s[tid / NG].gcount[tid % NG], c);
        }
        __syncthreads();
        for (int j = 0; j < 3 * NG; ++j) {
            const uint32_t c = min(scount[j], (uint32_t)kStage), base = sbase[j];
            V *L = lists + ((size_t)(3 * b + j / NG) * kLinLists + (j % NG)) * cap;
            for (uint32_t i = tid; i < c; i += 256)
                if (base + i < cap) L[base + i] = stg[j][i];
        }
        __syncthreads();
        if (tid < 3 * NG) scount[tid] = 0;
        __syncthreads();
    };
    constexpr int U = 2;
    for (int base = lo; base < hi; base += U * 1024) {
#pragma unroll
        for (int u = 0; u < U; ++u) {
            const int p = base + u * 1024 + tid * 4, m = min(4, hi - p);
            if (m > 0) {
                V r[3][4];
                if constexpr (sizeof(V) == 8) R.four64(p, m, r);
                else if (S.t32) R32.four(p, m, r);
                else R.four(p, m, r);
#pragma unroll
                for (int i = 0; i < 4; ++i) {
                    take(0, r[0][i], i < m);
                    take(1, r[1][i], i < m);
                    take(2, r[2][i], i < m);
                }
            }
        }
        flush(false);
    }
    flush(true);
}

template <typename V>
__global__ void __launch_bounds__(1024) k_lin_finish(const LinState *__restrict__ st, const V *__restrict__ lists,
                                                     uint32_t cap, V *__restrict__ os, uint32_t *__restrict__ flags, int pair,
                                                     int nlists)
{
    using K = typename Traits<V>::K;
    constexpr int kBuf = 49152 / (int)sizeof(V);
    __shared__ uint32_t h[2048], wsum[16], found[2], s_nloc;
    __shared__ unsigned long long s_kmin, s_kmax;
    __shared__ V s_buf[kBuf];
    const int bc = blockIdx.x, tid = threadIdx.x, lane = tid & 63;
    const LinState *s = st + bc;
    int q = blockIdx.y;
    if (pair) {
        const int half = (int)gridDim.y / 2;
        if (q < half) {
            q = 2 * q;
        } else {
            q = 2 * (q - half) + 1;
            if (s->gid[q] != kLinDone && s->gid[q] == s->gid[q - 1] && s->qbin[q] == s->qbin[q - 1] && s->rr[q] - s->rr[q - 1] <= 1u)
                return;
        }
    }
    const bool with_next = pair && !(q & 1);
    const uint32_t g = s->gid[q];
    if (g == kLinDone) return;
    const uint32_t cnt = s->gcount[g];
    if (cnt > cap) {
        if (tid == 0) flags[bc] = 1;
        return;
    }
    const V *L = lists + ((size_t)bc * nlists + g) * cap;
    uint32_t r = s->rr[q];
    const uint32_t tb = s->qbin[q];
    bool sub = false;
    float sub_lo = 0.0f, sub_scale = 0.0f;
    uint32_t sub_d = 0;
    auto subbin = [&](V x) -> uint32_t {
        const float f = ((float)x - sub_lo) * sub_scale;
        return (uint32_t)fminf(fmaxf(f, 0.0f), 2047.0f);
    };
    if (tb == kLinAnyBin && cnt > (uint32_t)kBuf) {
        sub = true;
        sub_lo = (float)(s->wlo[g] - 1u) * (1.0f / 2048.0f);
        sub_scale = 2048.0f * 2048.0f / (float)(s->wspan[g] + 1u);
        for (int i = tid; i < 2048; i += 1024) h[i] = 0;
        __syncthreads();
        constexpr int kFly = sizeof(V) == 4 ? 16 : 8;
        for (uint32_t base = 0; base < cnt; base += kFly * 1024) {
            V x[kFly];
#pragma unroll
            for (int u = 0; u < kFly; ++u) {
                const uint32_t i = min(base + u * 1024 + tid, cnt - 1);
                x[u] = L[i];
            }
#pragma unroll
            for (int u = 0; u < kFly; ++u)
                if (base + u * 1024 + tid < cnt) atomicAdd(&h[subbin(x[u])], 1u);
        }
        __syncthreads();
        uint32_t d, rr;
        block_find_digit(h, 2048, r, wsum, found, d, rr);
        sub_d = d;
        r = rr;
    }
    const uint32_t r_mine = r;
    auto is_mine = [&](V x, uint32_t i) -> bool {
        if (tb != kLinAnyBin) return lin_digit(x) == tb;
        return i < cnt && (!sub || subbin(x) == sub_d);
    };
    if (tid == 0) {
        s_nloc = 0;
        s_kmin = ~0ull;
        s_kmax = 0ull;
    }
    __syncthreads();
    {
        unsigned long long kmin = ~0ull, kmax = 0ull;
        constexpr int kFly = sizeof(V) == 4 ? 16 : 8;
        for (uint32_t base = 0; base < cnt; base += kFly * 1024) {
            V x[kFly];
#pragma unroll
            for (int u = 0; u < kFly; ++u) {
                const uint32_t i = base + u * 1024 + tid;
                const V v = L[min(i, cnt - 1)];
                x[u] = i < cnt ? v : (V)-1;
            }
#pragma unroll
            for (int u = 0; u < kFly; ++u) {
                const bool mine = is_mine(x[u], base + u * 1024 + tid);
                const uint64_t m = __ballot(mine);
                if (m) {
                    const int leader = (int)__builtin_ctzll(m);
                    uint32_t at = 0;
                    if (lane == leader) at = atomicAdd(&s_nloc, (uint32_t)__popcll(m));
                    at = __shfl(at, leader) + (uint32_t)__popcll(m & ((1ull << lane) - 1));
                    if (mine) {
                        const unsigned long long key = (unsigned long long)Traits<V>::key(x[u]);
                        kmin = key < kmin ? key : kmin;
                        kmax = key > kmax ? key : kmax;
                        if (at < (uint32_t)kBuf) s_buf[at] = x[u];
                    }
                }
            }
        }
#pragma unroll
        for (int o = 32; o > 0; o >>= 1) {
            const unsigned long long a = shfl_u64(kmin, lane ^ o), b = shfl_u64(kmax, lane ^ o);
            kmin = a < kmin ? a : kmin;
            kmax = b > kmax ? b : kmax;
        }
        if (lane == 0) {
            atomicMin(&s_kmin, kmin);
            atomicMax(&s_kmax, kmax);
        }
    }
    __syncthreads();
    const uint32_t nloc = s_nloc;
    const bool local = nloc <= (uint32_t)kBuf;
    const unsigned long long kmin = s_kmin, kmax = s_kmax;
    int lo = kmin == kmax ? 0 : 64 - __clzll((long long)(kmin ^ kmax));
    unsigned long long prefix = lo >= 64 ? 0ull : kmin >> lo;
    while (lo > 0) {
        const int bits = min(11, lo), shift = lo - bits, nbins = 1 << bits;
        for (int i = tid; i < nbins; i += 1024) h[i] = 0;
        __syncthreads();
        auto take = [&](V x, bool ok) {
            const unsigned long long key = (unsigned long long)Traits<V>::key(x);
            if (ok && (lo >= 64 || (key >> lo) == prefix)) atomicAdd(&h[(uint32_t)(key >> shift) & (uint32_t)(nbins - 1)], 1u);
        };
        if (local) {
            for (uint32_t i = tid; i < nloc; i += 1024) take(s_buf[i], true);
        } else {
            for (uint32_t base = 0; base < cnt; base += 8192) {
                V x[8];
#pragma unroll
                for (int u = 0; u < 8; ++u) {
                    const uint32_t i = base + u * 1024 + tid;
                    x[u] = i < cnt ? L[i] : (V)-1;
                }
#pragma unroll
                for (int u = 0; u < 8; ++u) take(x[u], is_mine(x[u], base + u * 1024 + tid));
            }
        }
        __syncthreads();
        uint32_t d, rr;
        block_find_digit(h, nbins, r, wsum, found, d, rr);
        prefix = (prefix << bits) | d;
        r = rr;
        lo = shift;
    }
    if (tid == 0) os[bc * kMaxRanks + q] = Traits<V>::value((K)prefix);
    if (!with_next) return;
    const int q1 = q + 1;
    if (s->gid[q1] != g || s->qbin[q1] != tb || s->rr[q1] - s->rr[q] > 1u) return;
    if (s->rr[q1] == s->rr[q]) {
        if (tid == 0) os[bc * kMaxRanks + q1] = Traits<V>::value((K)prefix);
        return;
    }
    __syncthreads();
    if (tid == 0) {
        s_nloc = 0;
        s_kmin = ~0ull;
    }
    __syncthreads();
    {
        uint32_t cle = 0;
        unsigned long long kgt = ~0ull;
        auto look = [&](V x, bool ok) {
            const unsigned long long key = (unsigned long long)Traits<V>::key(x);
            if (ok) {
                if (key <= prefix) ++cle;
                else kgt = key < kgt ? key : kgt;
            }
        };
        if (local) {
            for (uint32_t i = tid; i < nloc; i += 1024) look(s_buf[i], true);
        } else {
            for (uint32_t base = 0; base < cnt; base += 1024) {
                const uint32_t i = base + tid;
                const V x = i < cnt ? L[i] : (V)-1;
                look(x, is_mine(x, i));
            }
        }
        cle = wave_sum_u32(cle);
#pragma unroll
        for (int o = 32; o > 0; o >>= 1) {
            const unsigned long long a = shfl_u64(kgt, lane ^ o);
            kgt = a < kgt ? a : kgt;
        }
        if (lane == 0) {
            atomicAdd(&s_nloc, cle);
            atomicMin(&s_kmin, kgt);
        }
    }
    __syncthreads();
    if (sub && s_nloc <= r_mine + 1u && s_kmin == ~0ull) {
        unsigned long long kgt = ~0ull;
        for (uint32_t base = 0; base < cnt; base += 1024) {
            const uint32_t i = base + tid;
            if (i < cnt) {
                const unsigned long long key = (unsigned long long)Traits<V>::key(L[i]);
                if (key > prefix && key < kgt) kgt = key;
            }
        }
#pragma unroll
        for (int o = 32; o > 0; o >>= 1) {
            const unsigned long long a = shfl_u64(kgt, lane ^ o);
            kgt = a < kgt ? a : kgt;
        }
        if (lane == 0) atomicMin(&s_kmin, kgt);
        __syncthreads();
    }
    if (tid == 0) os[bc * kMaxRanks + q1] = Traits<V>::value((K)(s_nloc > r_mine + 1u ? prefix : s_kmin));
}

template <typename V>
struct LinRows;
template <>
struct LinRows<float> {
    static constexpr const char *sample = "k_lin_sample<float>", *scan = "k_lin_scan<float>", *collect = "k_lin_collect<float>",
                                *collect_src = "(k_lin_collect_src<float, 4>)", *finish = "k_lin_finish<float>";
};
template <>
struct LinRows<double> {
    static constexpr const char *sample = "k_lin_sample<double>", *scan = "k_lin_scan<double>", *collect = "k_lin_collect<double>",
                                *collect_src = "k_lin_collect_src64", *finish = "k_lin_finish<double>";
};

}

size_t select_ws_bytes(Shape s)
{
    Carver c(nullptr);
    SelectPlan plan;
    carve_select(c, s, true, &plan);
    return c.total();
}

template <typename V>
int select_lin_begin(Shape s, const double *q_percent, int nq, void *ws, hipStream_t st, SelectPlan *plan, const RestoreSrc *predict)
{
    constexpr bool f64 = sizeof(V) == 8;
    int rc = plan_percentiles<V>(s, q_percent, nq, ws, true, plan);
    if (rc == UWIE_OK) rc = zero_ghist(*plan, s, st);
    if (rc != UWIE_OK) return rc;
    const int n = (int)s.npx(), nbc = s.B * 3;
    const int ngroups = n / 4;
    plan->predicted = predict && !tune().lin_no_predict && (!f64 || (nq <= 2 && ngroups > 0));
    uint32_t ns = 0;
    if (plan->predicted && ngroups > 0) {
        int stride = std::max(1, ngroups / 32768);
        if (stride > 1) stride |= 1;
        const int ngs = ngroups / stride;
        ns = 4u * (uint32_t)ngs;
        UWIE_LAUNCH_AS(LinRows<V>::sample, k_lin_sample<V>, dim3(std::max(1, std::min(8, cdiv(ngs, 512))), s.B), dim3(256), 0, st,
                       *predict, n, stride, ngs, plan->ghist);
        UWIE_LAUNCH_CHECK();
    }
    UWIE_LAUNCH(k_lin_predict, dim3(nbc), dim3(256), 0, st, plan->lin, plan->ghist, rank_list(*plan), (uint32_t)n, ns,
                tune().lin_predict_shift);
    UWIE_LAUNCH_CHECK();
    return UWIE_OK;
}

template <typename V>
int select_lin_run(const SelectPlan &plan, const V *d_planar, Shape s, hipStream_t st, const RestoreSrc *src)
{
    using Rows = LinRows<V>;
    const int n = (int)s.npx(), nbc = s.B * 3;
    const RankList ranks = rank_list(plan);
    UWIE_REQUIRE(!src || ranks.n <= 4, "select_lin_run: the recomputing sweep handles at most two percentiles");
    V *lists = plan.lists_as<V>(), *os = (V *)plan.os;
    UWIE_LAUNCH_AS(Rows::scan, k_lin_scan<V>, dim3(nbc), dim3(256), 0, st, plan.lin, plan.ghist, ranks, os, plan.flags, plan.cap,
                   (SelState<typename Traits<V>::K> *)plan.state);
    UWIE_LAUNCH_CHECK();
    int blocks = (int)(((long long)n + 131071) / 131072);
    if (blocks * nbc < 1024) blocks = cdiv(1024, nbc);
    blocks = blocks < 1 ? 1 : blocks > 256 ? 256 : blocks;
    if (plan.predicted) blocks = std::max(1, std::min(2 * blocks, cdiv(24576, nbc)));
    if (src) {
        const int per_image = std::min(3 * blocks, std::max(1, cdiv(n, 2048)));
        UWIE_LAUNCH_AS(Rows::collect_src, (k_lin_collect_src<V, 4>), dim3(per_image, s.B), dim3(256), 0, st, *src, n, plan.lin, lists,
                       plan.cap);
    } else {
        UWIE_LAUNCH_AS(Rows::collect, k_lin_collect<V>, dim3(blocks, nbc), dim3(256), 0, st, d_planar, n, plan.lin, lists, plan.cap);
    }
    UWIE_LAUNCH_CHECK();
    UWIE_LAUNCH_AS(Rows::finish, k_lin_finish<V>, dim3(nbc, ranks.n), dim3(1024), 0, st, plan.lin, lists, plan.cap, os,
                   plan.flags, 0, kLinLists);
    UWIE_LAUNCH_CHECK();
    if (src) return sel_passes(plan, RestoredVals<V>{*src, n}, n, nbc, pass_blocks(n, nbc, true), false, plan.flags, st);
    const StoredVals<V> vals{d_planar, (size_t)n * 3, (size_t)n, 1};
    return sel_passes(plan, vals, n, nbc, pass_blocks(n, nbc, false), false, plan.flags, st);
}

template int select_lin_begin<float>(Shape, const double *, int, void *, hipStream_t, SelectPlan *, const RestoreSrc *);
template int select_lin_run<float>(const SelectPlan &, const float *, Shape, hipStream_t, const RestoreSrc *);
template int select_lin_begin<double>(Shape, const double *, int, void *, hipStream_t, SelectPlan *, const RestoreSrc *);
template int select_lin_run<double>(const SelectPlan &, const double *, Shape, hipStream_t, const RestoreSrc *);

int select_rank_run(const SelectPlan &plan, Shape s, hipStream_t st, const RestoreSrc &src)
{
    const int n = (int)s.npx(), nbc = s.B * 3;
    const RankList ranks = rank_list(plan);
    UWIE_LAUNCH(k_rank_scan, dim3(cdiv(nbc, 64)), dim3(64), 0, st, plan.lin, ranks, (float *)plan.os, plan.flags, kRankCapMul * plan.cap,
                nbc, (SelState<uint32_t> *)plan.state);
    UWIE_LAUNCH_CHECK();
    UWIE_LAUNCH(k_lin_finish<float>, dim3(nbc, ranks.n), dim3(1024), 0, st, plan.lin, plan.lists_as<float>(),
                kRankCapMul * plan.cap, (float *)plan.os, plan.flags, 1, kLinLists / kRankCapMul);
    UWIE_LAUNCH_CHECK();
    return sel_passes(plan, RestoredVals<float>{src, n}, n, nbc, pass_blocks(n, nbc, true), false, plan.flags, st);
}

int select_begin_stretch_ranks(Shape s, const float *d_params, int stride, void *ws, hipStream_t st, SelectPlan *plan)
{
    return begin_ranks(s, "stretch ranks: plane size out of range", ws, st, plan, [&](SelState<uint32_t> *state, int nbc, int n) {
        UWIE_LAUNCH(k_sel_init_stretch_ranks, dim3(cdiv(nbc, 64)), dim3(64), 0, st, state, nbc, d_params, stride, n);
    });
}

int select_begin_gated_ranks(Shape s, const float *d_params, int stride, uint32_t *d_status, void *ws, hipStream_t st,
                             SelectPlan *plan)
{
    return begin_ranks(s, "gated ranks: plane size out of range", ws, st, plan, [&](SelState<uint32_t> *state, int nbc, int n) {
        UWIE_LAUNCH(k_sel_init_gated_ranks, dim3(cdiv(nbc, 64)), dim3(64), 0, st, state, nbc, d_params, stride, n, d_status);
    });
}

int select_lerp_chain(const SelectPlan &plan, Shape s, float eps, float *d_pct4, hipStream_t st)
{
    UWIE_REQUIRE(plan.nq == 4 && !plan.is64, "chained stretch needs 4 float32 percentiles");
    FracList<float> fr;
    fr.n = 4;
    for (int j = 0; j < 4; ++j) fr.t[j] = (float)plan.t[j];
    const int nbc = s.B * 3;
    UWIE_LAUNCH(k_pct_finish_chain, dim3(cdiv(nbc, 64)), dim3(64), 0, st, (const float *)plan.os, nbc, fr, eps, d_pct4);
    UWIE_LAUNCH_CHECK();
    return UWIE_OK;
}

template <typename V>
int select_begin(Shape s, const double *q_percent, int nq, void *ws, hipStream_t st, SelectPlan *plan)
{
    using K = typename Traits<V>::K;
    const int rc = plan_percentiles<V>(s, q_percent, nq, ws, false, plan);
    if (rc != UWIE_OK) return rc;
    const int nbc = s.B * 3;
    UWIE_LAUNCH(k_sel_init<K>, dim3(cdiv(nbc, 64)), dim3(64), 0, st, (SelState<K> *)plan->state, nbc, rank_list(*plan));
    UWIE_LAUNCH_CHECK();
    return zero_ghist(*plan, s, st);
}

template <typename V>
int select_run(const SelectPlan &plan, const V *d_vals, int planar, Shape s, bool pass1_done, hipStream_t st)
{
    const int n = (int)s.npx(), nbc = s.B * 3;
    const StoredVals<V> src{d_vals, (size_t)n * 3, planar ? (size_t)n : (size_t)1, planar ? 1 : 3};
    return sel_passes(plan, src, n, nbc, pass_blocks(n, nbc, false), pass1_done, nullptr, st);
}

template <typename V>
int select_lerp(const SelectPlan &plan, Shape s, V *d_out, hipStream_t st)
{
    FracList<V> fr;
    fr.n = plan.nq;
    for (int j = 0; j < plan.nq; ++j) fr.t[j] = (V)plan.t[j];
    const int nbc = s.B * 3;
    UWIE_LAUNCH(k_pct_finish<V>, dim3(cdiv(nbc * plan.nq, 64)), dim3(64), 0, st, (const V *)plan.os, nbc, fr, d_out);
    UWIE_LAUNCH_CHECK();
    return UWIE_OK;
}

template <typename V>
int launch_percentiles(const V *d_vals, int planar, Shape s, const double *q_percent, int nq, V *d_out, void *ws, hipStream_t st)
{
    SelectPlan plan;
    int rc = select_begin<V>(s, q_percent, nq, ws, st, &plan);
    if (rc != UWIE_OK) return rc;
    rc = select_run(plan, d_vals, planar, s, false, st);
    if (rc != UWIE_OK) return rc;
    return select_lerp(plan, s, d_out, st);
}

template int select_begin<float>(Shape, const double *, int, void *, hipStream_t, SelectPlan *);
template int select_begin<double>(Shape, const double *, int, void *, hipStream_t, SelectPlan *);
template int select_run<float>(const SelectPlan &, const float *, int, Shape, bool, hipStream_t);
template int select_run<double>(const SelectPlan &, const double *, int, Shape, bool, hipStream_t);
template int select_lerp<float>(const SelectPlan &, Shape, float *, hipStream_t);
template int select_lerp<double>(const SelectPlan &, Shape, double *, hipStream_t);
template int launch_percentiles<float>(const float *, int, Shape, const double *, int, float *, void *, hipStream_t);
template int launch_percentiles<double>(const double *, int, Shape, const double *, int, double *, void *, hipStream_t);

// ... 18 lines not shown
```

underwater_image_enhancement_amd/runtime.py:

```python
from __future__ import annotations

import ctypes

import numpy as np
import torch

from . import _lib
from ._lib import UwieParams, check

_FRAME_DESC = np.dtype([("data", "<u8"), ("H", "<i4"), ("W", "<i4")])
_TRACE_DTYPE = np.dtype([("y0", "<i4"), ("x0", "<i4"), ("rows", "<i4"), ("cols", "<i4"), ("score", "<f8", (4,))])


def _ptr(t):
    return ctypes.c_void_p(t.data_ptr()) if t is not None else None


class _ClosedOnDel:

    def __del__(self):
        try:
            self.close()
        except Exception:
            pass
# ... 8 lines not shown
        self.index = int(device)
        self.torch_device = torch.device("cuda", self.index)
        torch.cuda.set_device(self.index)
        handle = ctypes.c_void_p()
        check(self.lib.uwie_create(self.index, ctypes.byref(handle)))
        self._ctx = handle
        self._workspace = None

    def close(self):
        if getattr(self, "_ctx", None):
            torch.cuda.synchronize(self.index)
            self.lib.uwie_destroy(self._ctx)
            self._ctx = None

    def stream(self):
        return ctypes.c_void_p(torch.cuda.current_stream(self.index).cuda_stream)

    def workspace(self, nbytes: int):
        if self._workspace is None or self._workspace.numel() < nbytes:
            self._workspace = None
            self._workspace = torch.empty(int(nbytes), dtype=torch.uint8, device=self.torch_device)
        return self._workspace

    def params(self, surface: int, strategy: int, **overrides) -> UwieParams:
        p = UwieParams()
        check(self.lib.uwie_params_init(ctypes.byref(p), surface, strategy))
        for key, value in overrides.items():
            if not hasattr(p, key):
                raise KeyError(key)
            setattr(p, key, value)
        return p

    def _sized_workspace(self, n: int, message: str, fresh: bool = False):
        if n == 0:
            raise _lib.UwieError(message)
        return torch.empty(int(n), dtype=torch.uint8, device=self.torch_device) if fresh else self.workspace(n)

    def workspace_for(self, B, H, W, p: UwieParams | None = None):
        n = self.lib.uwie_workspace_bytes_ctx(self._ctx, B, H, W, ctypes.byref(p) if p is not None else None)
        return self._sized_workspace(n, "batch/H/W out of range")

    def tensor(self, array, dtype=None):
        t = torch.as_tensor(np.ascontiguousarray(array))
        if dtype is not None:
            t = t.to(dtype)
        return t.to(self.torch_device)

    def empty(self, shape, dtype):
        return torch.empty(shape, dtype=dtype, device=self.torch_device)

    @staticmethod
    def _bhw(img):
        assert img.dim() == 4 and img.shape[-1] == 3 and img.is_contiguous(), "expected contiguous [B,H,W,3]"
        return int(img.shape[0]), int(img.shape[1]), int(img.shape[2])

    def tune(self, **selectors):
        for name, value in selectors.items():
            check(self.lib.uwie_set_tuning(self._ctx, name.encode(), int(value)))

    def tuning(self, **selectors):
        import contextlib

        @contextlib.contextmanager
        def scope():
            old = {}
            for name in selectors:
                v = ctypes.c_int()
                check(self.lib.uwie_get_tuning(self._ctx, name.encode(), ctypes.byref(v)))
                old[name] = v.value
            self.tune(**selectors)
            try:
                yield self
            finally:
                self.tune(**old)

        return scope()

    def check_status(self, allow: int = 0) -> int:
        bits = ctypes.c_uint32(0)
        rc = self.lib.uwie_device_status(self._ctx, self.stream(), ctypes.byref(bits))
        if rc != 0 and (bits.value == 0 or bits.value & ~allow):
            check(rc)
        return bits.value

    def profile(self, on: bool, only: str | None = None):
        check(self.lib.uwie_profile_filter(self._ctx, only.encode() if only else None))
        check(self.lib.uwie_profile_enable(self._ctx, int(bool(on))))

    def profile_rows(self):
        n = self.lib.uwie_profile_collect(self._ctx)
        if n < 0:
            check(n)
        rows = {}
        name, ms, calls = ctypes.c_char_p(), ctypes.c_double(), ctypes.c_int()
        for i in range(n):
            check(self.lib.uwie_profile_row(self._ctx, i, ctypes.byref(name), ctypes.byref(ms), ctypes.byref(calls)))
            rows[name.value.decode()] = (ms.value, calls.value)
        return rows

    def enhance_u8(self, frames, p: UwieParams, want_float: bool = False):
        B, H, W = self._bhw(frames)
        assert frames.dtype == torch.uint8
        ws = self.workspace_for(B, H, W, p)
        out = self.empty((B, H, W, 3), torch.uint8)
        outf = self.empty((B, H, W, 3), torch.float32) if want_float else None
        check(self.lib.uwie_enhance_u8(self._ctx, _ptr(frames), _ptr(out), _ptr(outf), B, H, W, ctypes.byref(p),
                                       _ptr(ws), ws.numel(), self.stream()))
        return out, outf

    def enhance_u8_f64(self, frames, p: UwieParams):
        B, H, W = self._bhw(frames)
        assert frames.dtype == torch.uint8
        ws = self.workspace_for(B, H, W, p)
        out = self.empty((B, H, W, 3), torch.uint8)
        outf = self.empty((B, H, W, 3), torch.float64)
        check(self.lib.uwie_enhance_u8_f64(self._ctx, _ptr(frames), _ptr(out), _ptr(outf), B, H, W, ctypes.byref(p),
                                           _ptr(ws), ws.numel(), self.stream()))
        return out, outf

    def enhance_percentiles(self, B, H, W, p: UwieParams):
        ws = self.workspace_for(B, H, W, p)
        k = 4 if p.surface == _lib.SURFACE_SIX and p.strategy == 3 else 2
        out = self.empty((B, 3, k), torch.float64)
        check(self.lib.uwie_enhance_percentiles(self._ctx, _ptr(ws), ws.numel(), B, H, W, ctypes.byref(p), _ptr(out),
                                                self.stream()))
        return out

    def enhance_u8_with_percentiles(self, frames, p: UwieParams, want_float: bool = False):
        out, outf = self.enhance_u8(frames, p, want_float)
        return out, outf, self.enhance_percentiles(*self._bhw(frames), p)

    def enhance_u8_f64_with_percentiles(self, frames, p: UwieParams):
        out, outf = self.enhance_u8_f64(frames, p)
        return out, outf, self.enhance_percentiles(*self._bhw(frames), p)

    def enhance_float(self, img, p: UwieParams, want: str = "native"):
        assert img.dim() == 4 and img.shape[-1] == 3 and img.is_contiguous(), "expected contiguous [B,H,W,3]"
        B, H, W = (int(v) for v in img.shape[:3])
        six = p.surface == _lib.SURFACE_SIX
        eb = 4 if img.dtype == torch.float32 else 8
        ws = self.workspace(self.lib.uwie_workspace_bytes_float(B, H, W, ctypes.byref(p), eb))
        out = self.empty((B, H, W, 3), torch.uint8)
        if img.dtype == torch.float32:
            of32 = self.empty((B, H, W, 3), torch.float32) if six else None
            of64 = None if six else self.empty((B, H, W, 3), torch.float64)
            check(self.lib.uwie_enhance_f32(self._ctx, _ptr(img), _ptr(out), _ptr(of32), _ptr(of64), B, H, W, ctypes.byref(p),
                                            _ptr(ws), ws.numel(), self.stream()))
            return out, (of32 if six else of64)
        assert img.dtype == torch.float64
        of64 = self.empty((B, H, W, 3), torch.float64)
        check(self.lib.uwie_enhance_f64(self._ctx, _ptr(img), _ptr(out), _ptr(of64), B, H, W, ctypes.byref(p), _ptr(ws),
                                        ws.numel(), self.stream()))
        return out, of64

    def cast_classify_f32(self, img):
        B, H, W = (int(v) for v in img.shape[:3])
        kind = self.empty((B,), torch.int32)
        mean = self.empty((B, 3), torch.float32)
        check(self.lib.uwie_cast_classify_f32(self._ctx, _ptr(img), B, H, W, _ptr(kind), _ptr(mean), self.stream()))
        return kind, mean

    def color_correct_f32(self, img, kind):
        B, H, W = (int(v) for v in img.shape[:3])
        out = self.empty((B, H, W, 3), torch.float32)
        check(self.lib.uwie_color_correct_f32(self._ctx, _ptr(img), _ptr(kind), _ptr(out), B, H, W, self.stream()))
        return out
# ... 608 lines not shown
```

Before: 59540.

## Use float-valued rank windows with finer sample histogram and dedicated rank finish kernel

Rank-based percentile selection now predicts windows from a finer 8192-bin sample histogram stored as float value bounds rather than coarse 2048-bin digits. Candidate lists shrink to two per channel, and a specialised finish kernel selects ranks from the list in LDS, reusing neighbouring ranks through a next-key scan. The intent is smaller candidate lists and less finishing work per plane. In exchange it adds a per-plane fallback counter and a larger shared-memory histogram in the sampling kernel.

```diff
diff --git a/include/uwie.h b/include/uwie.h
--- a/include/uwie.h
+++ b/include/uwie.h
@@ -69,6 +69,7 @@
 #define UWIE_STATUS_RESIZE_DESC 32u
 #define UWIE_STATUS_CLASSIFY_NAN 64u
 int uwie_device_status(uwie_ctx *ctx, void *stream, uint32_t *bits);
+int uwie_select_fallback_planes(uwie_ctx *ctx, void *stream, uint32_t *count);
 
 int uwie_profile_enable(uwie_ctx *ctx, int on);
 int uwie_profile_filter(uwie_ctx *ctx, const char *kernel_name);
diff --git a/underwater_image_enhancement_amd/_lib.py b/underwater_image_enhancement_amd/_lib.py
--- a/underwater_image_enhancement_amd/_lib.py
+++ b/underwater_image_enhancement_amd/_lib.py
@@ -142,6 +142,7 @@
     "uwie_create": [_I, ctypes.POINTER(_VP)],
     "uwie_destroy": [_VP],
     "uwie_device_status": [_VP, _VP, ctypes.POINTER(ctypes.c_uint32)],
+    "uwie_select_fallback_planes": [_VP, _VP, ctypes.POINTER(ctypes.c_uint32)],
     "uwie_profile_enable": [_VP, _I],
     "uwie_profile_filter": [_VP, ctypes.c_char_p],
     "uwie_profile_collect": [_VP],
diff --git a/underwater_image_enhancement_amd/csrc/api.hip b/underwater_image_enhancement_amd/csrc/api.hip
--- a/underwater_image_enhancement_amd/csrc/api.hip
+++ b/underwater_image_enhancement_amd/csrc/api.hip
@@ -297,8 +297,8 @@
         UWIE_TRY(launch_restore_planar_hist(d_in, kind, P.A, P.t, s, P.F, plan.ghist, st, false, nullptr, t_is_f32));
         UWIE_TRY(select_run(plan, P.F, 1, s, true, st));
     } else {
-        UWIE_TRY(select_lin_begin<float>(s, q, nq, P.scratch, st, &plan, e.predict ? &src : nullptr));
-        if (e.rank && plan.predicted) {
+        UWIE_TRY(select_lin_begin<float>(s, q, nq, P.scratch, st, &plan, e.predict ? &src : nullptr, e.rank));
+        if (plan.rank) {
             UWIE_TRY(launch_restore_rank(src, s, plan, st));
             UWIE_TRY(select_rank_run(plan, s, st, src));
         } else {
@@ -676,6 +676,18 @@
     return UWIE_OK;
 }
 
+int uwie_select_fallback_planes(uwie_ctx *ctx, void *stream, uint32_t *count)
+{
+    UWIE_REQUIRE(ctx && count, "select_fallback_planes: NULL pointer");
+    UWIE_SCOPE(ctx);
+    hipStream_t st = (hipStream_t)stream;
+    uint32_t *d = ctx->d_status + kStatusRankFallback;
+    UWIE_HIP_CHECK(hipMemcpyAsync(count, d, sizeof *count, hipMemcpyDeviceToHost, st));
+    UWIE_HIP_CHECK(hipStreamSynchronize(st));
+    if (*count) UWIE_HIP_CHECK(hipMemsetAsync(d, 0, sizeof *count, st));
+    return UWIE_OK;
+}
+
 int uwie_device_status_async(uwie_ctx *ctx, uint32_t *d_bits, void *stream)
 {
     UWIE_REQUIRE(ctx && d_bits, "device_status_async: NULL pointer");
diff --git a/underwater_image_enhancement_amd/csrc/common.h b/underwater_image_enhancement_amd/csrc/common.h
--- a/underwater_image_enhancement_amd/csrc/common.h
+++ b/underwater_image_enhancement_amd/csrc/common.h
@@ -101,6 +101,7 @@
 uwie_ctx *current_ctx();
 }
 
+constexpr int kStatusRankFallback = 1;
 struct uwie_ctx {
     int device;
     uwie::Tuning tune;
@@ -108,6 +109,7 @@
     bool attr_cast_resolve = false;
     int attr_gf_fast = 0;
     int attr_gf_split8 = 0;
+    bool attr_rank_finish = false;
     int cus = 0;
     uwie::LabTables *d_lab;
     uwie::CastTables *d_cast;
@@ -331,6 +333,8 @@
     uint32_t *flags;
     uint32_t cap;
     bool predicted;
+    bool rank;
+    uint32_t rank_cap;
     uint32_t ranks[2 * kMaxPct];
     template <typename V>
     V *lists_as() const { return static_cast<V *>(lists); }
@@ -359,15 +363,26 @@
     uint32_t gbin[2 * kMaxPct];
     uint32_t gcount[kLinLists];
     uint32_t ngroups;
-    uint32_t wlo[kMaxPct], wspan[kMaxPct];
+    union { uint32_t wlo[kMaxPct]; float vlo[kMaxPct]; };
+    union { uint32_t wspan[kMaxPct]; float vhi[kMaxPct]; };
     uint32_t below[kMaxPct];
 };
+constexpr int kRankNW = 2;
+constexpr int kRankSampleBins = 8192;
+__host__ __device__ inline int rank_side(float x, float vlo, float vhi)
+{
+    if (x < vlo || (vlo == 0.0f && x <= 0.0f)) return -1;
+    if (x > vhi || (vhi == 1.0f && x >= 1.0f)) return 1;
+    return 0;
+}
+__host__ __device__ inline bool rank_no_window(float vlo, float vhi) { return !(vlo <= vhi); }
+__host__ __device__ inline bool rank_below_is_zero(float vlo) { return vlo == 0.0f; }
+__host__ __device__ inline bool rank_above_is_one(float vhi) { return vhi == 1.0f; }
 constexpr int kRankCapMul = 4;
-constexpr uint32_t kLinAnyBin = 0xfffffffeu;
 struct RestoreSrc;
 template <typename V>
 int select_lin_begin(Shape s, const double *q_percent, int nq, void *ws, hipStream_t st, SelectPlan *plan,
-                     const RestoreSrc *predict = nullptr);
+                     const RestoreSrc *predict = nullptr, bool rank = false);
 template <typename V>
 int select_lin_run(const SelectPlan &plan, const V *d_planar, Shape s, hipStream_t st, const RestoreSrc *src = nullptr);
 template <typename V>
diff --git a/underwater_image_enhancement_amd/csrc/k_fused.hip b/underwater_image_enhancement_amd/csrc/k_fused.hip
--- a/underwater_image_enhancement_amd/csrc/k_fused.hip
+++ b/underwater_image_enhancement_amd/csrc/k_fused.hip
@@ -262,7 +262,7 @@
 }
 
 constexpr float kRankMargin = 1e-5f;
-constexpr int kRankNW = 2, kRankNS = 3 * kRankNW;
+constexpr int kRankNS = 3 * kRankNW;
 constexpr int kRankQW = 64 + 64 * 12;
 constexpr int kRankSW = 128;
 
@@ -271,7 +271,7 @@
     const double *t;
     const float *ftab;
     float a0, a1, a2;
-    const uint32_t *s_wlo, *s_wspan;
+    const float *s_vlo, *s_vhi;
     const float *s_lo, *s_hi;
     uint32_t *s_below;
     uint32_t *myq;
@@ -290,7 +290,7 @@
     uint32_t base = 0;
     if (X.lane == 0) base = atomicAdd(X.gcount0 + (size_t)c * X.gstride + w, n);
     base = (uint32_t)__builtin_amdgcn_readfirstlane((int)base);
-    float *L = X.lists0 + ((size_t)c * (kLinLists / kRankCapMul) + w) * X.cap;
+    float *L = X.lists0 + ((size_t)c * kRankNW + w) * X.cap;
     wave_lds_sync();
     for (uint32_t i = X.lane; i < n; i += 64)
         if (base + i < X.cap) L[base + i] = X.mystg[j][i];
@@ -318,16 +318,16 @@
             q = n / tv;
         }
         x = clip01((float)(q + (double)ac));
-        const uint32_t d = lin_digit(x);
         const float v32 = fmaf(df, __builtin_amdgcn_rcpf((float)tv), ac);
 #pragma unroll
         for (int w = 0; w < kRankNW; ++w) {
             const int j = c * kRankNW + w;
-            const uint32_t wlo = X.s_wlo[j];
-            if (wlo == kLinNoWin) continue;
+            const float vlo = X.s_vlo[j], vhi = X.s_vhi[j];
+            if (rank_no_window(vlo, vhi)) continue;
             if (counted && !(v32 >= X.s_lo[j] && v32 <= X.s_hi[j])) continue;
-            if (d < wlo) atomicAdd(&X.s_below[j], 1u);
-            else if (d - wlo <= X.s_wspan[j]) jj = j;
+            const int side = rank_side(x, vlo, vhi);
+            if (side < 0) atomicAdd(&X.s_below[j], 1u);
+            else if (side == 0) jj = j;
         }
     }
 #pragma unroll
@@ -349,18 +349,19 @@
     __shared__ uint32_t wq[4][QW];
     __shared__ float wstg[4][NS][SW];
     __shared__ float ftab[768];
-    __shared__ uint32_t s_wlo[NS], s_wspan[NS];
+    __shared__ float s_vlo[NS], s_vhi[NS];
     __shared__ float s_lo[NS], s_hi[NS];
     __shared__ uint32_t s_below[NS];
     const int b = blockIdx.y, tid = threadIdx.x, lane = tid & 63, wv = tid >> 6;
     if (tid < NS) {
         s_below[tid] = 0;
         const LinState &L = lin[3 * b + tid / NW];
-        const uint32_t lo = L.wlo[tid % NW], span = L.wspan[tid % NW];
-        s_wlo[tid] = lo;
-        s_wspan[tid] = span;
-        s_lo[tid] = lo == kLinNoWin ? __builtin_inff() : (float)(lo - 1) * (1.0f / 2048.0f) - kRankMargin;
-        s_hi[tid] = lo == kLinNoWin ? -__builtin_inff() : (float)(lo + span) * (1.0f / 2048.0f) + kRankMargin;
+        const float vlo = L.vlo[tid % NW], vhi = L.vhi[tid % NW];
+        const bool none = rank_no_window(vlo, vhi);
+        s_vlo[tid] = vlo;
+        s_vhi[tid] = vhi;
+        s_lo[tid] = none ? __builtin_inff() : vlo - kRankMargin;
+        s_hi[tid] = none ? -__builtin_inff() : vhi + kRankMargin;
     }
     RestoreImgT<1> R;
     R.init(S, b, (size_t)npx, ftab);
@@ -380,9 +381,9 @@
     uint32_t qn = 0;
     uint32_t sc[NS] = {0, 0, 0, 0, 0, 0};
 
-    const RankWave X{img, tpl, ftab, a0, a1, a2, s_wlo, s_wspan, s_lo, s_hi, s_below, myq, wstg[wv],
+    const RankWave X{img, tpl, ftab, a0, a1, a2, s_vlo, s_vhi, s_lo, s_hi, s_below, myq, wstg[wv],
                      &lin[3 * b].gcount[0], (uint32_t)(sizeof(LinState) / sizeof(uint32_t)),
-                     lists + (size_t)(3 * b) * (kLinLists / kRankCapMul) * cap, cap, lane};
+                     lists + (size_t)(3 * b) * kRankNW * cap, cap, lane};
 
     const int step = gridDim.x * 1024, iters = (npx + step - 1) / step;
 #define UWIE_RANK_LOAD4(p_, w_, tv_)                                                                                   \
@@ -1304,9 +1305,9 @@
 
 int launch_restore_rank(const RestoreSrc &src, Shape s, const SelectPlan &plan, hipStream_t st)
 {
-    UWIE_REQUIRE(!src.t32 && plan.nq <= 2 && plan.predicted && s.npx() >= 4, "restore_rank: float64 transmission, two predicted percentiles");
+    UWIE_REQUIRE(!src.t32 && plan.nq <= kRankNW && plan.rank && s.npx() >= 4, "restore_rank: float64 transmission, two predicted percentiles");
     UWIE_LAUNCH(k_restore_rank, dim3(producer_blocks(5120, s), s.B), dim3(256), 0, st, src, (int)s.npx(), plan.lin, plan.lists_as<float>(),
-                (uint32_t)kRankCapMul * plan.cap);
+                plan.rank_cap);
     UWIE_LAUNCH_CHECK();
     return UWIE_OK;
 }
diff --git a/underwater_image_enhancement_amd/csrc/k_select.hip b/underwater_image_enhancement_amd/csrc/k_select.hip
--- a/underwater_image_enhancement_amd/csrc/k_select.hip
+++ b/underwater_image_enhancement_amd/csrc/k_select.hip
@@ -406,6 +406,8 @@
     plan->lin = c.take<LinState>(nbc);
     plan->flags = c.take<uint32_t>(nbc);
     plan->cap = lin_cap(s);
+    plan->rank_cap = (uint32_t)kRankCapMul * plan->cap;
+    plan->rank = false;
     plan->lists = c.take<double>(nbc * kLinLists * plan->cap);
 }
 
@@ -522,6 +524,102 @@
     }
 }
 
+__device__ __forceinline__ uint32_t rank_sample_bin(float x)
+{
+    return min((uint32_t)(clamp01(x) * (float)kRankSampleBins), (uint32_t)kRankSampleBins - 1u);
+}
+__global__ void __launch_bounds__(256) k_lin_sample_rank(RestoreSrc S, int npx, int stride, int ngs, uint32_t *__restrict__ ghist)
+{
+    constexpr int kWords = kRankSampleBins / 2;
+    __shared__ uint32_t h[3][kWords];
+    const int b = blockIdx.y, tid = threadIdx.x;
+    for (int i = tid; i < 3 * kWords; i += 256) (&h[0][0])[i] = 0;
+    __syncthreads();
+    RestoreImg R;
+    R.init(S, b, (size_t)npx);
+    for (int i = blockIdx.x * 256 + tid; i < ngs; i += gridDim.x * 256) {
+        float r[3][4];
+        R.four((i * stride + stride / 2) * 4, 4, r);
+#pragma unroll
+        for (int c = 0; c < 3; ++c)
+#pragma unroll
+            for (int j = 0; j < 4; ++j) {
+                const uint32_t d = rank_sample_bin(r[c][j]);
+                atomicAdd(&h[c][d >> 1], 1u << (16 * (d & 1u)));
+            }
+    }
+    __syncthreads();
+    for (int i = tid; i < 3 * kWords; i += 256) {
+        const uint32_t w = (&h[0][0])[i];
+        uint32_t *g = ghist + (size_t)(b * 3 + i / kWords) * kSelGroupStride + kLinSampleOff + 2 * (i % kWords);
+        if (w & 0xffffu) atomicAdd(g, w & 0xffffu);
+        if (w >> 16) atomicAdd(g + 1, w >> 16);
+    }
+}
+
+__device__ void merge_windows(uint32_t *wl, uint32_t *wh)
+{
+    for (bool again = true; again;) {
+        again = false;
+        for (int i = 0; i < kMaxPct; ++i)
+            for (int j = i + 1; j < kMaxPct; ++j)
+                if (wl[i] != kLinNoWin && wl[j] != kLinNoWin && wl[j] <= wh[i] + 1 && wl[i] <= wh[j] + 1) {
+                    wl[i] = min(wl[i], wl[j]);
+                    wh[i] = max(wh[i], wh[j]);
+                    wl[j] = kLinNoWin;
+                    again = true;
+                }
+    }
+}
+
+__device__ __forceinline__ void sample_rank_range(const RankList &ranks, int j, uint32_t n, uint32_t ns, uint32_t &rlo, uint32_t &rhi)
+{
+    const double p = (double)ranks.r[2 * j] / (double)n, sd = sqrt((double)ns * p * (1.0 - p));
+    const double c0 = (double)ranks.r[2 * j] * ns / n, c1 = (double)ranks.r[2 * j + 1] * ns / n, delta = 4.0 * sd + 2.0;
+    rlo = (uint32_t)fmax(c0 - delta, 0.0);
+    rhi = (uint32_t)fmin(c1 + delta, (double)ns - 1.0);
+}
+
+__global__ void __launch_bounds__(256) k_lin_predict_rank(LinState *__restrict__ st, uint32_t *__restrict__ ghist, RankList ranks,
+                                                          uint32_t n, uint32_t ns, int shift)
+{
+    constexpr int NB = kRankSampleBins;
+    __shared__ uint32_t h[NB], wsum[4], found[2], wl[kMaxPct], wh[kMaxPct];
+    const int bc = blockIdx.x, tid = threadIdx.x;
+    if (tid < kMaxPct) { wl[tid] = kLinNoWin; wh[tid] = 0; }
+    uint32_t *gh = ghist + (size_t)bc * kSelGroupStride + kLinSampleOff;
+    for (int i = tid; i < NB; i += 256) {
+        h[i] = gh[i];
+        gh[i] = 0;
+    }
+    __syncthreads();
+    for (int j = 0; j < ranks.n / 2 && j < kRankNW; ++j) {
+        uint32_t rlo, rhi, dlo, dhi, rr;
+        sample_rank_range(ranks, j, n, ns, rlo, rhi);
+        block_find_digit(h, NB, rlo, wsum, found, dlo, rr);
+        block_find_digit(h, NB, rhi, wsum, found, dhi, rr);
+        if (tid == 0) {
+            wl[j] = (uint32_t)min(max((int)dlo + shift * (NB / 2048), 0), NB - 1);
+            wh[j] = (uint32_t)min(max((int)dhi + shift * (NB / 2048), (int)wl[j]), NB - 1);
+        }
+    }
+    __syncthreads();
+    if (tid == 0) {
+        LinState s;
+        for (int q = 0; q < kMaxRanks; ++q) { s.rr[q] = 0; s.qbin[q] = 0; s.gid[q] = kLinDone; s.gbin[q] = kLinDone; }
+        for (int g = 0; g < kLinLists; ++g) s.gcount[g] = 0;
+        s.ngroups = 0;
+        merge_windows(wl, wh);
+        for (int w = 0; w < kMaxPct; ++w) {
+            const bool none = wl[w] == kLinNoWin;
+            s.vlo[w] = none ? __builtin_inff() : (float)wl[w] * (1.0f / NB);
+            s.vhi[w] = none ? -__builtin_inff() : (float)(wh[w] + 1u) * (1.0f / NB);
+            s.below[w] = 0;
+        }
+        st[bc] = s;
+    }
+}
+
 __global__ void __launch_bounds__(256) k_lin_predict(LinState *__restrict__ st, uint32_t *__restrict__ ghist,
                                                      RankList ranks, uint32_t n, uint32_t ns, int shift)
 {
@@ -536,10 +634,8 @@
         }
         __syncthreads();
         for (int j = 0; j < ranks.n / 2 && j < kMaxPct; ++j) {
-            const double p = (double)ranks.r[2 * j] / (double)n, sd = sqrt((double)ns * p * (1.0 - p));
-            const double c0 = (double)ranks.r[2 * j] * ns / n, c1 = (double)ranks.r[2 * j + 1] * ns / n, delta = 4.0 * sd + 2.0;
-            const uint32_t rlo = (uint32_t)fmax(c0 - delta, 0.0), rhi = (uint32_t)fmin(c1 + delta, (double)ns - 1.0);
-            uint32_t dlo, dhi, rr;
+            uint32_t rlo, rhi, dlo, dhi, rr;
+            sample_rank_range(ranks, j, n, ns, rlo, rhi);
             block_find_digit(h, kLinBins, rlo, wsum, found, dlo, rr);
             block_find_digit(h, kLinBins, rhi, wsum, found, dhi, rr);
             if (tid == 0) {
@@ -554,17 +650,7 @@
         for (int q = 0; q < kMaxRanks; ++q) { s.rr[q] = 0; s.qbin[q] = 0; s.gid[q] = kLinDone; s.gbin[q] = kLinDone; }
         for (int g = 0; g < kLinLists; ++g) s.gcount[g] = 0;
         s.ngroups = 0;
-        for (bool again = true; again;) {
-            again = false;
-            for (int i = 0; i < kMaxPct; ++i)
-                for (int j = i + 1; j < kMaxPct; ++j)
-                    if (wl[i] != kLinNoWin && wl[j] != kLinNoWin && wl[j] <= wh[i] + 1 && wl[i] <= wh[j] + 1) {
-                        wl[i] = min(wl[i], wl[j]);
-                        wh[i] = max(wh[i], wh[j]);
-                        wl[j] = kLinNoWin;
-                        again = true;
-                    }
-        }
+        merge_windows(wl, wh);
         for (int w = 0; w < kMaxPct; ++w) {
             s.wlo[w] = wl[w];
             s.wspan[w] = wl[w] == kLinNoWin ? 0 : wh[w] - wl[w];
@@ -632,7 +718,7 @@
 }
 
 __global__ void k_rank_scan(LinState *__restrict__ st, RankList ranks, float *__restrict__ os, uint32_t *__restrict__ flags,
-                            uint32_t cap, int nbc, SelState<uint32_t> *__restrict__ sel)
+                            uint32_t cap, int nbc, SelState<uint32_t> *__restrict__ sel, uint32_t *__restrict__ nflagged)
 {
     const int bc = blockIdx.x * blockDim.x + threadIdx.x;
     if (bc >= nbc) return;
@@ -644,21 +730,20 @@
         const uint32_t r = ranks.r[q];
         bool done = false;
         for (int w = 0; w < kMaxPct && !done; ++w) {
-            if (s.wlo[w] == kLinNoWin) continue;
+            if (rank_no_window(s.vlo[w], s.vhi[w])) continue;
             const uint32_t below = s.below[w], cnt = s.gcount[w];
             if (r >= below && r - below < cnt) {
                 if (cnt <= cap) {
                     s.gid[q] = (uint32_t)w;
                     s.rr[q] = r - below;
-                    s.qbin[q] = kLinAnyBin;
                 } else {
                     miss = true;
                 }
                 done = true;
-            } else if (r < below && s.wlo[w] == 1u) {
+            } else if (r < below && rank_below_is_zero(s.vlo[w])) {
                 os[bc * kMaxRanks + q] = 0.0f;
                 done = true;
-            } else if (r >= below && s.wlo[w] + s.wspan[w] == (uint32_t)kLinBins - 2u) {
+            } else if (r >= below && rank_above_is_one(s.vhi[w])) {
                 os[bc * kMaxRanks + q] = 1.0f;
                 done = true;
             }
@@ -668,6 +753,7 @@
     s.ngroups = 0;
     st[bc] = s;
     flags[bc] = miss ? 1u : 0u;
+    if (miss && nflagged) atomicAdd(nflagged, 1u);
 }
 
 template <typename V>
@@ -845,8 +931,7 @@
 
 template <typename V>
 __global__ void __launch_bounds__(1024) k_lin_finish(const LinState *__restrict__ st, const V *__restrict__ lists,
-                                                     uint32_t cap, V *__restrict__ os, uint32_t *__restrict__ flags, int pair,
-                                                     int nlists)
+                                                     uint32_t cap, V *__restrict__ os, uint32_t *__restrict__ flags)
 {
     using K = typename Traits<V>::K;
     constexpr int kBuf = 49152 / (int)sizeof(V);
@@ -855,18 +940,7 @@
     __shared__ V s_buf[kBuf];
     const int bc = blockIdx.x, tid = threadIdx.x, lane = tid & 63;
     const LinState *s = st + bc;
-    int q = blockIdx.y;
-    if (pair) {
-        const int half = (int)gridDim.y / 2;
-        if (q < half) {
-            q = 2 * q;
-        } else {
-            q = 2 * (q - half) + 1;
-            if (s->gid[q] != kLinDone && s->gid[q] == s->gid[q - 1] && s->qbin[q] == s->qbin[q - 1] && s->rr[q] - s->rr[q - 1] <= 1u)
-                return;
-        }
-    }
-    const bool with_next = pair && !(q & 1);
+    const int q = blockIdx.y;
     const uint32_t g = s->gid[q];
     if (g == kLinDone) return;
     const uint32_t cnt = s->gcount[g];
@@ -874,45 +948,10 @@
         if (tid == 0) flags[bc] = 1;
         return;
     }
-    const V *L = lists + ((size_t)bc * nlists + g) * cap;
+    const V *L = lists + ((size_t)bc * kLinLists + g) * cap;
     uint32_t r = s->rr[q];
     const uint32_t tb = s->qbin[q];
-    bool sub = false;
-    float sub_lo = 0.0f, sub_scale = 0.0f;
-    uint32_t sub_d = 0;
-    auto subbin = [&](V x) -> uint32_t {
-        const float f = ((float)x - sub_lo) * sub_scale;
-        return (uint32_t)fminf(fmaxf(f, 0.0f), 2047.0f);
-    };
-    if (tb == kLinAnyBin && cnt > (uint32_t)kBuf) {
-        sub = true;
-        sub_lo = (float)(s->wlo[g] - 1u) * (1.0f / 2048.0f);
-        sub_scale = 2048.0f * 2048.0f / (float)(s->wspan[g] + 1u);
-        for (int i = tid; i < 2048; i += 1024) h[i] = 0;
-        __syncthreads();
-        constexpr int kFly = sizeof(V) == 4 ? 16 : 8;
-        for (uint32_t base = 0; base < cnt; base += kFly * 1024) {
-            V x[kFly];
-#pragma unroll
-            for (int u = 0; u < kFly; ++u) {
-                const uint32_t i = min(base + u * 1024 + tid, cnt - 1);
-                x[u] = L[i];
-            }
-#pragma unroll
-            for (int u = 0; u < kFly; ++u)
-                if (base + u * 1024 + tid < cnt) atomicAdd(&h[subbin(x[u])], 1u);
-        }
-        __syncthreads();
-        uint32_t d, rr;
-        block_find_digit(h, 2048, r, wsum, found, d, rr);
-        sub_d = d;
-        r = rr;
-    }
-    const uint32_t r_mine = r;
-    auto is_mine = [&](V x, uint32_t i) -> bool {
-        if (tb != kLinAnyBin) return lin_digit(x) == tb;
-        return i < cnt && (!sub || subbin(x) == sub_d);
-    };
+    auto is_mine = [&](V x) -> bool { return lin_digit(x) == tb; };
     if (tid == 0) {
         s_nloc = 0;
         s_kmin = ~0ull;
@@ -932,7 +971,7 @@
             }
 #pragma unroll
             for (int u = 0; u < kFly; ++u) {
-                const bool mine = is_mine(x[u], base + u * 1024 + tid);
+                const bool mine = is_mine(x[u]);
                 const uint64_t m = __ballot(mine);
                 if (m) {
                     const int leader = (int)__builtin_ctzll(m);
@@ -984,7 +1023,7 @@
                     x[u] = i < cnt ? L[i] : (V)-1;
                 }
 #pragma unroll
-                for (int u = 0; u < 8; ++u) take(x[u], is_mine(x[u], base + u * 1024 + tid));
+                for (int u = 0; u < 8; ++u) take(x[u], is_mine(x[u]));
             }
         }
         __syncthreads();
@@ -995,68 +1034,126 @@
         lo = shift;
     }
     if (tid == 0) os[bc * kMaxRanks + q] = Traits<V>::value((K)prefix);
-    if (!with_next) return;
-    const int q1 = q + 1;
-    if (s->gid[q1] != g || s->qbin[q1] != tb || s->rr[q1] - s->rr[q] > 1u) return;
-    if (s->rr[q1] == s->rr[q]) {
-        if (tid == 0) os[bc * kMaxRanks + q1] = Traits<V>::value((K)prefix);
-        return;
-    }
-    __syncthreads();
+}
+
+constexpr int kRankBuf = 32768;
+__global__ void __launch_bounds__(1024) k_lin_finish_rank(const LinState *__restrict__ st, const float *__restrict__ lists,
+                                                          uint32_t cap, float *__restrict__ os, int nq)
+{
+    __shared__ uint32_t h[2048], wsum[16], found[2], s_cle, s_kmin, s_kmax;
+    extern __shared__ float s_buf[];
+    const int bc = blockIdx.x, w = blockIdx.y, tid = threadIdx.x, lane = tid & 63;
+    const LinState *s = st + bc;
+    bool any = false;
+    for (int q = 0; q < nq; ++q) any = any || s->gid[q] == (uint32_t)w;
+    if (!any) return;
+    const uint32_t cnt = s->gcount[w];
+    const float *L = lists + ((size_t)bc * kRankNW + w) * cap;
+    const bool local = cnt <= (uint32_t)kRankBuf;
+    constexpr int kFly = 16;
+    auto each = [&](auto &&f) {
+        for (uint32_t base = 0; base < cnt; base += kFly * 1024) {
+            float x[kFly];
+#pragma unroll
+            for (int u = 0; u < kFly; ++u) {
+                const uint32_t i = min(base + u * 1024 + tid, cnt - 1);
+                x[u] = local ? s_buf[i] : L[i];
+            }
+#pragma unroll
+            for (int u = 0; u < kFly; ++u)
+                if (base + u * 1024 + tid < cnt) f(f32_key(x[u]));
+        }
+    };
     if (tid == 0) {
-        s_nloc = 0;
-        s_kmin = ~0ull;
+        s_kmin = 0xffffffffu;
+        s_kmax = 0u;
     }
     __syncthreads();
     {
-        uint32_t cle = 0;
-        unsigned long long kgt = ~0ull;
-        auto look = [&](V x, bool ok) {
-            const unsigned long long key = (unsigned long long)Traits<V>::key(x);
-            if (ok) {
-                if (key <= prefix) ++cle;
-                else kgt = key < kgt ? key : kgt;
-            }
-        };
-        if (local) {
-            for (uint32_t i = tid; i < nloc; i += 1024) look(s_buf[i], true);
-        } else {
-            for (uint32_t base = 0; base < cnt; base += 1024) {
-                const uint32_t i = base + tid;
-                const V x = i < cnt ? L[i] : (V)-1;
-                look(x, is_mine(x, i));
-            }
-        }
+        uint32_t kmin = 0xffffffffu, kmax = 0u;
+        for (uint32_t base = 0; base < cnt; base += kFly * 1024) {
+            float x[kFly];
+#pragma unroll
+            for (int u = 0; u < kFly; ++u) x[u] = L[min(base + u * 1024 + tid, cnt - 1)];
+#pragma unroll
+            for (int u = 0; u < kFly; ++u) {
+                const uint32_t i = base + u * 1024 + tid;
+                if (i < cnt) {
+                    const uint32_t key = f32_key(x[u]);
+                    kmin = min(kmin, key);
+                    kmax = max(kmax, key);
+                    if (local) s_buf[i] = x[u];
+                }
+            }
+        }
+#pragma unroll
+        for (int o = 32; o > 0; o >>= 1) {
+            kmin = min(kmin, (uint32_t)__shfl_xor((int)kmin, o));
+            kmax = max(kmax, (uint32_t)__shfl_xor((int)kmax, o));
+        }
+        if (lane == 0) {
+            atomicMin(&s_kmin, kmin);
+            atomicMax(&s_kmax, kmax);
+        }
+    }
+    __syncthreads();
+    const uint32_t kmin = s_kmin, kmax = s_kmax;
+    const int nbits = kmin == kmax ? 0 : 32 - __clz((int)(kmin ^ kmax));
+    auto select = [&](uint32_t r) -> uint32_t {
+        int lo = nbits;
+        uint32_t prefix = lo >= 32 ? 0u : kmin >> lo;
+        while (lo > 0) {
+            const int bits = min(11, lo), shift = lo - bits, nbins = 1 << bits;
+            for (int i = tid; i < nbins; i += 1024) h[i] = 0;
+            __syncthreads();
+            each([&](uint32_t key) {
+                if (lo >= 32 || (key >> lo) == prefix) atomicAdd(&h[(key >> shift) & (uint32_t)(nbins - 1)], 1u);
+            });
+            __syncthreads();
+            uint32_t d, rr;
+            block_find_digit(h, nbins, r, wsum, found, d, rr);
+            prefix = (prefix << bits) | d;
+            r = rr;
+            lo = shift;
+        }
+        return prefix;
+    };
+    auto next = [&](uint32_t key_r, uint32_t r) -> uint32_t {
+        __syncthreads();
+        if (tid == 0) {
+            s_cle = 0;
+            s_kmin = 0xffffffffu;
+        }
+        __syncthreads();
+        uint32_t cle = 0, kgt = 0xffffffffu;
+        each([&](uint32_t key) {
+            if (key <= key_r) ++cle;
+            else kgt = min(kgt, key);
+        });
         cle = wave_sum_u32(cle);
 #pragma unroll
-        for (int o = 32; o > 0; o >>= 1) {
-            const unsigned long long a = shfl_u64(kgt, lane ^ o);
-            kgt = a < kgt ? a : kgt;
-        }
+        for (int o = 32; o > 0; o >>= 1) kgt = min(kgt, (uint32_t)__shfl_xor((int)kgt, o));
         if (lane == 0) {
-            atomicAdd(&s_nloc, cle);
+            atomicAdd(&s_cle, cle);
             atomicMin(&s_kmin, kgt);
         }
-    }
-    __syncthreads();
-    if (sub && s_nloc <= r_mine + 1u && s_kmin == ~0ull) {
-        unsigned long long kgt = ~0ull;
-        for (uint32_t base = 0; base < cnt; base += 1024) {
-            const uint32_t i = base + tid;
-            if (i < cnt) {
-                const unsigned long long key = (unsigned long long)Traits<V>::key(L[i]);
-                if (key > prefix && key < kgt) kgt = key;
-            }
-        }
-#pragma unroll
-        for (int o = 32; o > 0; o >>= 1) {
-            const unsigned long long a = shfl_u64(kgt, lane ^ o);
-            kgt = a < kgt ? a : kgt;
-        }
-        if (lane == 0) atomicMin(&s_kmin, kgt);
-        __syncthreads();
-    }
-    if (tid == 0) os[bc * kMaxRanks + q1] = Traits<V>::value((K)(s_nloc > r_mine + 1u ? prefix : s_kmin));
+        __syncthreads();
+        return s_cle > r + 1u ? key_r : s_kmin;
+    };
+    bool have = false;
+    uint32_t r_prev = 0, key_prev = 0;
+    for (int q = 0; q < nq; ++q) {
+        if (s->gid[q] != (uint32_t)w) continue;
+        const uint32_t r = s->rr[q];
+        uint32_t key;
+        if (have && r == r_prev) key = key_prev;
+        else if (have && r == r_prev + 1u) key = next(key_prev, r_prev);
+        else key = select(r);
+        if (tid == 0) os[bc * kMaxRanks + q] = Traits<float>::value(key);
+        have = true;
+        r_prev = r;
+        key_prev = key;
+    }
 }
 
 template <typename V>
@@ -1083,7 +1180,8 @@
 }
 
 template <typename V>
-int select_lin_begin(Shape s, const double *q_percent, int nq, void *ws, hipStream_t st, SelectPlan *plan, const RestoreSrc *predict)
+int select_lin_begin(Shape s, const double *q_percent, int nq, void *ws, hipStream_t st, SelectPlan *plan, const RestoreSrc *predict,
+                     bool rank)
 {
     constexpr bool f64 = sizeof(V) == 8;
     int rc = plan_percentiles<V>(s, q_percent, nq, ws, true, plan);
@@ -1092,18 +1190,26 @@
     const int n = (int)s.npx(), nbc = s.B * 3;
     const int ngroups = n / 4;
     plan->predicted = predict && !tune().lin_no_predict && (!f64 || (nq <= 2 && ngroups > 0));
+    plan->rank = !f64 && rank && plan->predicted && !predict->t32 && ngroups > 0 && nq <= kRankNW;
     uint32_t ns = 0;
     if (plan->predicted && ngroups > 0) {
         int stride = std::max(1, ngroups / 32768);
         if (stride > 1) stride |= 1;
         const int ngs = ngroups / stride;
         ns = 4u * (uint32_t)ngs;
-        UWIE_LAUNCH_AS(LinRows<V>::sample, k_lin_sample<V>, dim3(std::max(1, std::min(8, cdiv(ngs, 512))), s.B), dim3(256), 0, st,
-                       *predict, n, stride, ngs, plan->ghist);
+        const dim3 grid(std::max(1, std::min(8, cdiv(ngs, 512))), s.B);
+        if constexpr (!f64) {
+            if (plan->rank) UWIE_LAUNCH_AS(LinRows<V>::sample, k_lin_sample_rank, grid, dim3(256), 0, st, *predict, n, stride, ngs, plan->ghist);
+        }
+        if (!plan->rank) UWIE_LAUNCH_AS(LinRows<V>::sample, k_lin_sample<V>, grid, dim3(256), 0, st, *predict, n, stride, ngs, plan->ghist);
         UWIE_LAUNCH_CHECK();
     }
-    UWIE_LAUNCH(k_lin_predict, dim3(nbc), dim3(256), 0, st, plan->lin, plan->ghist, rank_list(*plan), (uint32_t)n, ns,
-                tune().lin_predict_shift);
+    if (plan->rank)
+        UWIE_LAUNCH_AS("k_lin_predict", k_lin_predict_rank, dim3(nbc), dim3(256), 0, st, plan->lin, plan->ghist, rank_list(*plan),
+                       (uint32_t)n, ns, tune().lin_predict_shift);
+    else
+        UWIE_LAUNCH(k_lin_predict, dim3(nbc), dim3(256), 0, st, plan->lin, plan->ghist, rank_list(*plan), (uint32_t)n, ns,
+                    tune().lin_predict_shift);
     UWIE_LAUNCH_CHECK();
     return UWIE_OK;
 }
@@ -1132,27 +1238,34 @@
     }
     UWIE_LAUNCH_CHECK();
     UWIE_LAUNCH_AS(Rows::finish, k_lin_finish<V>, dim3(nbc, ranks.n), dim3(1024), 0, st, plan.lin, lists, plan.cap, os,
-                   plan.flags, 0, kLinLists);
+                   plan.flags);
     UWIE_LAUNCH_CHECK();
     if (src) return sel_passes(plan, RestoredVals<V>{*src, n}, n, nbc, pass_blocks(n, nbc, true), false, plan.flags, st);
     const StoredVals<V> vals{d_planar, (size_t)n * 3, (size_t)n, 1};
     return sel_passes(plan, vals, n, nbc, pass_blocks(n, nbc, false), false, plan.flags, st);
 }
 
-template int select_lin_begin<float>(Shape, const double *, int, void *, hipStream_t, SelectPlan *, const RestoreSrc *);
+template int select_lin_begin<float>(Shape, const double *, int, void *, hipStream_t, SelectPlan *, const RestoreSrc *, bool);
 template int select_lin_run<float>(const SelectPlan &, const float *, Shape, hipStream_t, const RestoreSrc *);
-template int select_lin_begin<double>(Shape, const double *, int, void *, hipStream_t, SelectPlan *, const RestoreSrc *);
+template int select_lin_begin<double>(Shape, const double *, int, void *, hipStream_t, SelectPlan *, const RestoreSrc *, bool);
 template int select_lin_run<double>(const SelectPlan &, const double *, Shape, hipStream_t, const RestoreSrc *);
 
 int select_rank_run(const SelectPlan &plan, Shape s, hipStream_t st, const RestoreSrc &src)
 {
     const int n = (int)s.npx(), nbc = s.B * 3;
     const RankList ranks = rank_list(plan);
-    UWIE_LAUNCH(k_rank_scan, dim3(cdiv(nbc, 64)), dim3(64), 0, st, plan.lin, ranks, (float *)plan.os, plan.flags, kRankCapMul * plan.cap,
-                nbc, (SelState<uint32_t> *)plan.state);
+    uwie_ctx *ctx = current_ctx();
+    UWIE_LAUNCH(k_rank_scan, dim3(cdiv(nbc, 64)), dim3(64), 0, st, plan.lin, ranks, (float *)plan.os, plan.flags, plan.rank_cap, nbc,
+                (SelState<uint32_t> *)plan.state, ctx ? ctx->d_status + kStatusRankFallback : nullptr);
     UWIE_LAUNCH_CHECK();
-    UWIE_LAUNCH(k_lin_finish<float>, dim3(nbc, ranks.n), dim3(1024), 0, st, plan.lin, plan.lists_as<float>(),
-                kRankCapMul * plan.cap, (float *)plan.os, plan.flags, 1, kLinLists / kRankCapMul);
+    constexpr size_t kFinishLds = (size_t)kRankBuf * sizeof(float);
+    if (!ctx || !ctx->attr_rank_finish) {
+        UWIE_HIP_CHECK(hipFuncSetAttribute(reinterpret_cast<const void *>(k_lin_finish_rank), hipFuncAttributeMaxDynamicSharedMemorySize,
+                                           (int)kFinishLds));
+        if (ctx) ctx->attr_rank_finish = true;
+    }
+    UWIE_LAUNCH_AS(LinRows<float>::finish, k_lin_finish_rank, dim3(nbc, kRankNW), dim3(1024), kFinishLds, st, plan.lin,
+                   plan.lists_as<float>(), plan.rank_cap, (float *)plan.os, ranks.n);
     UWIE_LAUNCH_CHECK();
     return sel_passes(plan, RestoredVals<float>{src, n}, n, nbc, pass_blocks(n, nbc, true), false, plan.flags, st);
 }
diff --git a/underwater_image_enhancement_amd/runtime.py b/underwater_image_enhancement_amd/runtime.py
--- a/underwater_image_enhancement_amd/runtime.py
+++ b/underwater_image_enhancement_amd/runtime.py
@@ -114,6 +114,11 @@
         if rc != 0 and (bits.value == 0 or bits.value & ~allow):
             check(rc)
         return bits.value
+
+    def select_fallback_planes(self) -> int:
+        count = ctypes.c_uint32(0)
+        check(self.lib.uwie_select_fallback_planes(self._ctx, self.stream(), ctypes.byref(count)))
+        return count.value
 
     def profile(self, on: bool, only: str | None = None):
         check(self.lib.uwie_profile_filter(self._ctx, only.encode() if only else None))
```

Measured after the change: 59350, median of 2. About the same (-0.3%).
